# hamaadshah/gan_deeplearning4j

Measured on NVIDIA H100. Metric: images/sec (full G+D step), higher is better.
Workload: dtype bf16

## Files before the change

gan_deeplearning4j_b200/_lib.py:

```python
from __future__ import annotations

import ctypes as C
import os

_HERE = os.path.dirname(os.path.abspath(__file__))
LIB_PATH = os.path.join(_HERE, "lib", "libb200gan.so")
NAME_LEN = 64


class B200GanError(RuntimeError):
    def __init__(self, code, msg):
        super().__init__(f"libb200gan error {code}: {msg}")
        self.code = code


class LayerDesc(C.Structure):
    _fields_ = [("type", C.c_int32), ("name", C.c_char * NAME_LEN), ("n_in", C.c_int32), ("n_out", C.c_int32),
                ("k_h", C.c_int32), ("k_w", C.c_int32), ("s_h", C.c_int32), ("s_w", C.c_int32), ("p_h", C.c_int32), ("p_w", C.c_int32),
                ("has_bias", C.c_int32), ("act", C.c_int32), ("act_alpha", C.c_float), ("updater", C.c_int32),
                ("lr", C.c_float), ("beta1", C.c_float), ("beta2", C.c_float), ("eps", C.c_float), ("l2", C.c_float),
                ("bn_decay", C.c_float), ("bn_eps", C.c_float), ("pre_h", C.c_int32), ("pre_w", C.c_int32), ("pre_c", C.c_int32),
                ("loss", C.c_int32), ("frozen", C.c_int32)]


class NetConfig(C.Structure):
    _fields_ = [("in_h", C.c_int32), ("in_w", C.c_int32), ("in_c", C.c_int32), ("max_batch", C.c_int32), ("precision", C.c_int32),
                ("grad_clip", C.c_float), ("xent_clip_eps", C.c_float), ("bn_groups", C.c_int32), ("seed", C.c_uint64)]


class GanConfig(C.Structure):
    _fields_ = [("fake_bn_train", C.c_int32), ("use_cuda_graph", C.c_int32)]


class LrSchedule(C.Structure):
    _fields_ = [("kind", C.c_int32), ("type", C.c_int32), ("initial", C.c_double), ("gamma", C.c_double), ("power", C.c_double),
                ("step", C.c_double), ("decay_rate", C.c_double), ("n_map", C.c_int32), ("map_keys", C.POINTER(C.c_int32)),
                ("map_values", C.POINTER(C.c_double))]


class ConvGeom(C.Structure):
    _fields_ = [(k, C.c_int32) for k in ("n", "h", "w", "c", "oh", "ow", "o", "kh", "kw", "sh", "sw", "ph", "pw")]


class TestConvOpts(C.Structure):
    _fields_ = [("epi", C.c_int32), ("act", C.c_int32), ("alpha", C.c_float), ("bias", C.POINTER(C.c_float)), ("scale", C.POINTER(C.c_float)),
                ("groups", C.c_int32), ("aux", C.POINTER(C.c_float)), ("aux2", C.POINTER(C.c_float)), ("stats", C.POINTER(C.c_double)), ("kernel", C.c_char * 64),
                ("bn", C.c_int32), ("max_ctas", C.c_int32), ("poison", C.c_int32), ("w_mn", C.c_int32), ("per_tap", C.c_int32), ("slab", C.c_int32),
                ("defer", C.c_int32), ("db", C.POINTER(C.c_float)), ("param_offset", C.c_int32), ("splits", C.c_int32)]


class EwReduceJob(C.Structure):
    _fields_ = [("n", C.c_int64), ("stride", C.c_int64), ("src_off", C.c_int64), ("dst_off", C.c_int64), ("splits", C.c_int32), ("wide", C.c_int32)]


class TestEwOpts(C.Structure):
    _fields_ = [("op", C.c_int32), ("n", C.c_int64), ("rows", C.c_int32), ("cols", C.c_int32), ("groups", C.c_int32), ("splits", C.c_int32),
                ("stride", C.c_int64)] + [(k, C.c_int32) for k in ("N", "H", "W", "C", "KH", "KW", "SH", "SW", "act")] + [
                ("alpha", C.c_float), ("clip_eps", C.c_float), ("offset", C.c_int32), ("in_place", C.c_int32), ("accumulate", C.c_int32),
                ("poison", C.c_int32), ("n_jobs", C.c_int32), ("jobs", C.POINTER(EwReduceJob)), ("n_seg", C.c_int32),
                ("seg_off", C.POINTER(C.c_int64)), ("seg_len", C.POINTER(C.c_int64)), ("seg_coef", C.POINTER(C.c_float)), ("sumsq", C.c_double),
                ("kernel", C.c_char * 64), ("loss", C.c_int32)]


class TestPoolOpts(C.Structure):
    _fields_ = [("op", C.c_int32), ("pool", C.c_int32), ("pnorm", C.c_float)] + [
                (k, C.c_int32) for k in ("N", "H", "W", "C", "KH", "KW", "SH", "SW", "PH", "PW", "offset", "poison")] + [
                ("kernel", C.c_char * 64), ("splits", C.c_int32)]


_vp, _i32, _i64, _fp = C.c_void_p, C.c_int32, C.c_int64, C.POINTER(C.c_float)
_pvp = C.POINTER(C.c_void_p)

PROTOTYPES = {
    "b2g_version": (_i32, []),
    "b2g_ctx_create": (_i32, [_i32, _pvp]),
    "b2g_ctx_destroy": (_i32, [_vp]),
    "b2g_last_error": (C.c_char_p, []),
    "b2g_sync": (_i32, [_vp]),
    "b2g_launch_count": (_i32, [_vp, C.POINTER(C.c_uint64)]),
    "b2g_timer_start": (_i32, [_vp]),
    "b2g_timer_stop_ms": (_i32, [_vp, _fp]),
    "b2g_flush_l2": (_i32, [_vp]),
    "b2g_device_info": (_i32, [_vp, C.POINTER(_i32), C.POINTER(_i32), C.POINTER(_i32), C.POINTER(C.c_uint64)]),
    "b2g_net_create": (_i32, [_vp, C.POINTER(NetConfig), C.POINTER(LayerDesc), _i32, _pvp]),
    "b2g_net_destroy": (_i32, [_vp]),
    "b2g_net_num_params": (_i32, [_vp, C.POINTER(_i64)]),
    "b2g_net_output_size": (_i32, [_vp, C.POINTER(_i64)]),
    "b2g_net_layer_output_size": (_i32, [_vp, _i32, C.POINTER(_i64)]),
    "b2g_net_set_param": (_i32, [_vp, C.c_char_p, C.c_char_p, _fp, _i64]),
    "b2g_net_get_param": (_i32, [_vp, C.c_char_p, C.c_char_p, _fp, _i64]),
    "b2g_net_get_params": (_i32, [_vp, _fp, _i64]),
    "b2g_net_set_params": (_i32, [_vp, _fp, _i64]),
    "b2g_net_get_gradients": (_i32, [_vp, _fp, _i64]),
    "b2g_net_updater_state_size": (_i32, [_vp, C.POINTER(_i64)]),
    "b2g_net_get_updater_state": (_i32, [_vp, _fp, _i64]),
    "b2g_net_set_updater_state": (_i32, [_vp, _fp, _i64]),
    "b2g_net_output": (_i32, [_vp, _fp, _i32, _i32, _fp]),
    "b2g_net_get_activation": (_i32, [_vp, _i32, _i32, _fp]),
    "b2g_net_compute_gradient_and_score": (_i32, [_vp, _fp, _fp, _i32, _fp]),
    "b2g_net_get_input_gradient": (_i32, [_vp, _i32, _fp]),
    "b2g_net_fit": (_i32, [_vp, _fp, _fp, _i32, _fp]),
    "b2g_net_get_iteration": (_i32, [_vp, C.POINTER(_i64)]),
    "b2g_net_set_iteration": (_i32, [_vp, _i64]),
    "b2g_net_get_dropout_pass": (_i32, [_vp, C.POINTER(_i64)]),
    "b2g_net_set_dropout_pass": (_i32, [_vp, _i64]),
    "b2g_net_set_gradient_normalization": (_i32, [_vp, _i32, C.c_float]),
    "b2g_net_set_lr_schedule": (_i32, [_vp, C.c_char_p, C.POINTER(LrSchedule)]),
    "b2g_net_get_learning_rate": (_i32, [_vp, C.c_char_p, _fp]),
    "b2g_net_get_epoch": (_i32, [_vp, C.POINTER(_i64)]),
    "b2g_net_set_epoch": (_i32, [_vp, _i64]),
    "b2g_net_simt_gemm_calls": (_i32, [_vp, C.POINTER(C.c_uint64)]),
    "b2g_gan_create": (_i32, [_vp, _vp, C.POINTER(GanConfig), _pvp]),
    "b2g_gan_destroy": (_i32, [_vp]),
    "b2g_gan_step": (_i32, [_vp, _fp, _fp, _fp, _fp, _fp, _fp, _i32, _fp]),
    "b2g_gan_upload": (_i32, [_vp, _fp, _fp, _fp, _fp, _fp, _fp, _i32]),
    "b2g_gan_step_resident": (_i32, [_vp, _i32]),
    "b2g_gan_read_losses": (_i32, [_vp, _fp]),
    "b2g_gan_last_step_ms": (_i32, [_vp, _fp]),
    "b2g_comm_unique_id": (_i32, [_vp]),
    "b2g_ctx_comm_init": (_i32, [_vp, _i32, _i32, _vp]),
    "b2g_ctx_comm_destroy": (_i32, [_vp]),
    "b2g_net_set_grad_allreduce": (_i32, [_vp, _i32]),
    "b2g_net_average_parameters": (_i32, [_vp]),
    "b2g_net_set_sync_bn": (_i32, [_vp, _i32]),
    "b2g_net_set_grad_payload_bf16": (_i32, [_vp, _i32]),
    "b2g_net_enable_p2p_allreduce": (_i32, [_vp, C.POINTER(C.c_int32)]),
    "b2g_ctx_allreduce_test": (_i32, [_vp, _fp, _i64]),
    "b2g_test_conv": (_i32, [_vp, _i32, _i32, _i32, C.POINTER(ConvGeom), _fp, _fp, _fp, _i32, _fp]),
    "b2g_test_hbm_kernels": (_i32, [_vp, _i32, _i32, _i32, _fp]),
    "b2g_test_conv_ex": (_i32, [_vp, _i32, _i32, _i32, C.POINTER(ConvGeom), _fp, _fp, _fp, _i32, _fp, C.POINTER(TestConvOpts)]),
    "b2g_test_bn": (_i32, [_vp, _i32, _i32, _i32, _i32, _i32, _fp, _fp, _fp, _fp, _fp, _fp, _i32, C.c_float, C.c_float, C.c_float,
                           _i32, _fp, _fp, _fp, _fp, _fp, _fp, _fp, _fp]),
    "b2g_test_net_shadow": (_i32, [_vp, _i32, _i32, _fp, _i64]),
    "b2g_test_dropout": (_i32, [_vp, _i32, C.c_uint64, _i32, _i32, _i64, _i32, _i32, _i32, _i32, C.c_float, _fp, _fp, _fp, _fp]),
    "b2g_test_ew": (_i32, [_vp, _i32, C.POINTER(TestEwOpts), _fp, _fp, _fp, _fp, _fp]),
    "b2g_test_pool": (_i32, [_vp, _i32, C.POINTER(TestPoolOpts), _fp, _fp, _fp, _fp, _fp]),
}

_lib = None


def load():
    global _lib
    if _lib is not None:
        return _lib
    if not os.path.exists(LIB_PATH):
        raise B200GanError(-7, f"{LIB_PATH} is missing: build it with `make` (nvcc, sm_90a). There is no CPU fallback.")
    lib = C.CDLL(LIB_PATH, mode=C.RTLD_GLOBAL)
    for name, (res, args) in PROTOTYPES.items():
        fn = getattr(lib, name)
        fn.restype, fn.argtypes = res, args
    _lib = lib
    return lib


def check(code):
    if code != 0:
        raise B200GanError(code, load().b2g_last_error().decode(errors="replace"))
```

gan_deeplearning4j_b200/csrc/engine.cu:

```cuda
#include <cuda_runtime.h>
#include <dlfcn.h>
#include <math.h>
#include <stdarg.h>
#include <stdio.h>
#include <stdlib.h>
#include <string.h>

#include <algorithm>
#include <string>
#include <vector>

#include "../../include/b200gan.h"
#include "kernels.h"

using namespace b2g;

static thread_local char g_err[1024] = "";
static int32_t fail(int32_t code, const char* fmt, ...) {
  va_list ap; va_start(ap, fmt); vsnprintf(g_err, sizeof(g_err), fmt, ap); va_end(ap); return code;
}
#define CU(call) do { cudaError_t e_ = (call); if (e_ != cudaSuccess) return fail(B2G_ERR_CUDA, "%s:%d %s -> %s", __FILE__, __LINE__, #call, cudaGetErrorString(e_)); } while (0)
#define B2(call) do { int32_t r_ = (call); if (r_ != 0) return r_; } while (0)
#define CHECK_KERNELS() CU(cudaGetLastError())

// ... 1202 lines not shown
}
static bool layer_has_lr(const b2g_net* n, int li) { return lr_segment(n, li) >= 0; }
static int32_t find_lr_layer(const b2g_net* n, const char* layer, int* li) {
  for (size_t i = 0; i < n->L.size(); ++i) if (!strncmp(n->L[i].d.name, layer, B2G_NAME_LEN)) {
    if (!layer_has_lr(n, (int)i)) return fail(B2G_ERR_ARG, "layer %s has no learning rate (frozen, no parameters, NoOp or AdaDelta)", layer);
    *li = (int)i; return 0;
  }
  return fail(B2G_ERR_ARG, "no layer named %s", layer);
}
static int32_t net_upload_schedules(b2g_net* n) {
  cudaStream_t s = n->ctx->stream;
  size_t nv = 0; for (auto& ls : n->layer_sched) nv += ls.vals.size();
  const size_t bytes = nv * (sizeof(double) + sizeof(int32_t));
  CU(cudaStreamSynchronize(s));
  if (bytes > n->sched_map_bytes) {
    if (n->sched_map) { cudaFree(n->sched_map); n->sched_map = nullptr; n->sched_map_bytes = 0; }
    cudaError_t e = cudaMalloc(&n->sched_map, bytes);
    if (e != cudaSuccess) { n->sched_map = nullptr; return fail(B2G_ERR_OOM, "cudaMalloc(%zu) failed: %s", bytes, cudaGetErrorString(e)); }
    n->sched_map_bytes = bytes;
  }
  std::vector<char> host(bytes); double* dv = (double*)n->sched_map; int32_t* dk = (int32_t*)((char*)n->sched_map + nv * sizeof(double));
  std::vector<UpdSched> per_layer(n->L.size()); size_t at = 0;
  for (size_t li = 0; li < n->L.size(); ++li) {
    const auto& ls = n->layer_sched[li]; per_layer[li] = ls.sc;
    if (ls.sc.kind == B2G_SCHED_MAP) {
      memcpy(host.data() + at * sizeof(double), ls.vals.data(), ls.vals.size() * sizeof(double));
      memcpy(host.data() + nv * sizeof(double) + at * sizeof(int32_t), ls.keys.data(), ls.keys.size() * sizeof(int32_t));
      per_layer[li].vals = dv + at; per_layer[li].keys = dk + at; at += ls.vals.size();
    }
  }
  std::vector<UpdSched> seg(n->segs.size()); bool on = false;
  for (size_t i = 0; i < n->segs.size(); ++i) { seg[i] = per_layer[n->seg_layer[i]]; on = on || seg[i].kind != B2G_SCHED_NONE; }
  if (bytes) CU(cudaMemcpyAsync(n->sched_map, host.data(), bytes, cudaMemcpyHostToDevice, s));
  if (!seg.empty()) CU(cudaMemcpyAsync(n->sched_dev, seg.data(), sizeof(UpdSched) * seg.size(), cudaMemcpyHostToDevice, s));
  CU(cudaStreamSynchronize(s));
  n->sched_on = on; ++n->settings_gen;
  return 0;
}
extern "C" int32_t b2g_net_set_lr_schedule(b2g_net* n, const char* layer, const b2g_lr_schedule* s) {
  if (!n) return fail(B2G_ERR_ARG, "null"); CU(cudaSetDevice(n->ctx->device));
  b2g_net::LayerSched ls;
  if (s && s->kind != B2G_SCHED_NONE) {
    if (s->kind < B2G_SCHED_EXPONENTIAL || s->kind > B2G_SCHED_MAP) return fail(B2G_ERR_ARG, "unknown schedule kind %d (PolySchedule is not supported)", s->kind);
    if (s->type != B2G_SCHED_ITERATION && s->type != B2G_SCHED_EPOCH) return fail(B2G_ERR_ARG, "unknown schedule type %d", s->type);
    if (!std::isfinite(s->initial) || !std::isfinite(s->gamma) || !std::isfinite(s->power) || !std::isfinite(s->step) || !std::isfinite(s->decay_rate))
      return fail(B2G_ERR_ARG, "schedule parameters must be finite");
    if (s->kind == B2G_SCHED_STEP && !(s->step > 0.0)) return fail(B2G_ERR_ARG, "StepSchedule step %g: must be > 0", s->step);
    if (s->kind == B2G_SCHED_INVERSE && s->gamma < 0.0) return fail(B2G_ERR_ARG, "InverseSchedule gamma %g: must be >= 0", s->gamma);
    UpdSched& sc = ls.sc; sc.kind = s->kind; sc.type = s->type;
    sc.initial = s->initial; sc.gamma = s->gamma; sc.power = s->power; sc.step = s->step; sc.decay = s->decay_rate;
    if (s->kind == B2G_SCHED_MAP) {
      if (s->n_map < 1 || !s->map_keys || !s->map_values) return fail(B2G_ERR_ARG, "MapSchedule needs at least one entry");
      bool has0 = false;
      for (int j = 0; j < s->n_map; ++j) {
        if (j > 0 && s->map_keys[j] <= s->map_keys[j - 1]) return fail(B2G_ERR_ARG, "MapSchedule keys must strictly increase");
        if (!std::isfinite(s->map_values[j])) return fail(B2G_ERR_ARG, "MapSchedule values must be finite");
        has0 = has0 || s->map_keys[j] == 0;
      }
      if (!has0) return fail(B2G_ERR_ARG, "MapSchedule has no value for key 0");
      ls.keys.assign(s->map_keys, s->map_keys + s->n_map); ls.vals.assign(s->map_values, s->map_values + s->n_map); sc.n_map = s->n_map;
    }
  }
  if (layer) { int li = 0; B2(find_lr_layer(n, layer, &li)); n->layer_sched[li] = ls; }
  else for (size_t li = 0; li < n->L.size(); ++li) if (layer_has_lr(n, (int)li)) n->layer_sched[li] = ls;
  return net_upload_schedules(n);
}
extern "C" int32_t b2g_net_get_learning_rate(b2g_net* n, const char* layer, float* out) {
  if (!n || !layer || !out) return fail(B2G_ERR_ARG, "null"); CU(cudaSetDevice(n->ctx->device));
  int li = 0; B2(find_lr_layer(n, layer, &li));
  const int seg = lr_segment(n, li);
  k_sched_lr(n->segs_dev, n->sched_dev, seg, n->step_dev, n->epoch_dev, n->lr_out, n->ctx->stream); CHECK_KERNELS();
  CU(cudaMemcpyAsync(out, n->lr_out, sizeof(float), cudaMemcpyDeviceToHost, n->ctx->stream)); CU(cudaStreamSynchronize(n->ctx->stream));
  return 0;
}
extern "C" int32_t b2g_net_get_epoch(b2g_net* n, int64_t* out) {
  if (!n || !out) return fail(B2G_ERR_ARG, "null"); CU(cudaSetDevice(n->ctx->device));
  int64_t v = 0; CU(cudaMemcpyAsync(&v, n->epoch_dev, sizeof(v), cudaMemcpyDeviceToHost, n->ctx->stream)); CU(cudaStreamSynchronize(n->ctx->stream)); *out = v; return 0;
}
extern "C" int32_t b2g_net_set_epoch(b2g_net* n, int64_t epoch) {
  if (!n || epoch < 0) return fail(B2G_ERR_ARG, "bad epoch"); CU(cudaSetDevice(n->ctx->device));
  CU(cudaMemcpyAsync(n->epoch_dev, &epoch, sizeof(epoch), cudaMemcpyHostToDevice, n->ctx->stream)); CU(cudaStreamSynchronize(n->ctx->stream)); return 0;
}
extern "C" int32_t b2g_net_simt_gemm_calls(b2g_net* n, uint64_t* out) { if (!n || !out) return fail(B2G_ERR_ARG, "null"); *out = n->simt_gemm_calls; return 0; }

extern "C" int32_t b2g_comm_unique_id(void* id128) { if (!id128) return fail(B2G_ERR_ARG, "null"); B2(nccl_load()); NcclId id; NC(g_nccl.uid(&id)); memcpy(id128, &id, sizeof(id)); return 0; }
extern "C" int32_t b2g_ctx_comm_init(b2g_ctx* c, int32_t world, int32_t rank, const void* id128) {
  if (!c || !id128 || world < 1 || rank < 0 || rank >= world) return fail(B2G_ERR_ARG, "bad communicator arguments");
  B2(nccl_load()); CU(cudaSetDevice(c->device));
  NcclId id; memcpy(&id, id128, sizeof(id));
  NC(g_nccl.init(&c->comm, world, id, rank)); c->world = world; c->rank = rank; return 0;
}
extern "C" int32_t b2g_ctx_comm_destroy(b2g_ctx* c) { if (c && c->comm) { g_nccl.destroy(c->comm); c->comm = nullptr; c->world = 1; c->rank = 0; } return 0; }
extern "C" int32_t b2g_net_set_grad_allreduce(b2g_net* n, int32_t enabled) { if (!n) return fail(B2G_ERR_ARG, "null"); n->grad_allreduce = enabled != 0; return 0; }
extern "C" int32_t b2g_net_set_sync_bn(b2g_net* n, int32_t enabled) { if (!n) return fail(B2G_ERR_ARG, "null"); if (enabled && n->prec != PREC_BF16) return fail(B2G_ERR_UNSUPPORTED, "sync_bn rides on the fused BatchNorm path (BF16 nets)"); n->sync_bn = enabled != 0; return 0; }
extern "C" int32_t b2g_net_set_grad_payload_bf16(b2g_net* n, int32_t enabled) {
  if (!n) return fail(B2G_ERR_ARG, "null"); CU(cudaSetDevice(n->ctx->device));
  if (enabled && !n->ar_buf) B2(dalloc(n, &n->ar_buf, sizeof(__nv_bfloat16) * (size_t)n->n_params));
  n->ar_bf16 = enabled != 0; return 0;
}
extern "C" int32_t b2g_net_enable_p2p_allreduce(b2g_net* n, int32_t* enabled) {
  if (!n) return fail(B2G_ERR_ARG, "null"); b2g_ctx* c = n->ctx; CU(cudaSetDevice(c->device)); if (enabled) *enabled = 0;
  if (!c->comm || c->world < 2) return 0;
  if (c->world > 8 || !g_nccl.ag) return 0;
  cudaStream_t s = c->stream;
  if (!c->p2p_flags) { CU(cudaMalloc(&c->p2p_flags, 16 * sizeof(unsigned))); CU(cudaMalloc(&c->p2p_state, 2 * sizeof(unsigned)));
                       CU(cudaMemsetAsync(c->p2p_flags, 0, 16 * sizeof(unsigned), s)); CU(cudaMemsetAsync(c->p2p_state, 0, 2 * sizeof(unsigned), s)); CU(cudaStreamSynchronize(s)); }
  struct Pair { cudaIpcMemHandle_t flags, grads; };
  Pair mine; memset(&mine, 0, sizeof(mine)); float ok = 1.f;
  if (cudaIpcGetMemHandle(&mine.flags, c->p2p_flags) != cudaSuccess || cudaIpcGetMemHandle(&mine.grads, n->grads) != cudaSuccess) { cudaGetLastError(); ok = 0.f; }
  std::vector<Pair> all(c->world);
  char *d_send = nullptr, *d_recv = nullptr; float* d_ok = nullptr;
  CU(cudaMalloc(&d_send, sizeof(Pair))); CU(cudaMalloc(&d_recv, sizeof(Pair) * c->world)); CU(cudaMalloc(&d_ok, sizeof(float)));
  CU(cudaMemcpyAsync(d_send, &mine, sizeof(Pair), cudaMemcpyHostToDevice, s));
  NC(g_nccl.ag(d_send, d_recv, sizeof(Pair),  0, c->comm, s));
  CU(cudaMemcpyAsync(all.data(), d_recv, sizeof(Pair) * c->world, cudaMemcpyDeviceToHost, s)); CU(cudaStreamSynchronize(s));
  float* pg[8] = {}; unsigned* pf[8] = {};
  for (int r = 0; r < c->world && ok > 0.f; ++r) {
    if (r == c->rank) { pg[r] = n->grads; pf[r] = c->p2p_flags; continue; }
    void* q = nullptr;
    if (cudaIpcOpenMemHandle(&q, all[r].grads, cudaIpcMemLazyEnablePeerAccess) != cudaSuccess) { cudaGetLastError(); ok = 0.f; break; }
    pg[r] = (float*)q;
    if (c->p2p_flags_mapped) pf[r] = c->p2p_peer_flags[r];
    else { if (cudaIpcOpenMemHandle(&q, all[r].flags, cudaIpcMemLazyEnablePeerAccess) != cudaSuccess) { cudaGetLastError(); ok = 0.f; break; } pf[r] = (unsigned*)q; }
  }
  CU(cudaMemcpyAsync(d_ok, &ok, sizeof(float), cudaMemcpyHostToDevice, s)); NC(g_nccl.ar(d_ok, d_ok, 1, 7, 0, c->comm, s));
  float sum = 0.f; CU(cudaMemcpyAsync(&sum, d_ok, sizeof(float), cudaMemcpyDeviceToHost, s)); CU(cudaStreamSynchronize(s));
  cudaFree(d_send); cudaFree(d_recv); cudaFree(d_ok);
  if (sum < (float)c->world - 0.5f) {
    for (int r = 0; r < c->world; ++r) { if (r == c->rank) continue; if (pg[r]) cudaIpcCloseMemHandle(pg[r]); if (!c->p2p_flags_mapped && pf[r]) cudaIpcCloseMemHandle(pf[r]); }
    return 0;
  }
  for (int r = 0; r < c->world; ++r) { n->p2p_peer_grads[r] = pg[r]; c->p2p_peer_flags[r] = pf[r]; }
  c->p2p_flags_mapped = true; n->p2p = true; if (enabled) *enabled = 1;
  return 0;
}
extern "C" int32_t b2g_net_average_parameters(b2g_net* n) {
  if (!n) return fail(B2G_ERR_ARG, "null"); b2g_ctx* c = n->ctx; CU(cudaSetDevice(c->device));
  if (!c->comm || c->world == 1) return 0;
  const float inv = 1.0f / (float)c->world; cudaStream_t s = c->stream;
  float* bufs[4] = {n->params, n->st0, n->st1, n->st2};
  for (float* b : bufs) { if (!b) continue; NC(g_nccl.ar(b, b, (size_t)n->n_params, 7, 0, c->comm, s)); k_scale_f32(b, inv, (size_t)n->n_params, s); }
  net_refresh_shadow(n);
  CU(cudaStreamSynchronize(s)); return 0;
}
extern "C" int32_t b2g_ctx_allreduce_test(b2g_ctx* c, float* host, int64_t n) {
  if (!c || !host || n < 1) return fail(B2G_ERR_ARG, "null"); if (!c->comm) return fail(B2G_ERR_NCCL, "no communicator"); CU(cudaSetDevice(c->device));
  float* d = nullptr; CU(cudaMalloc(&d, sizeof(float) * n));
  CU(cudaMemcpyAsync(d, host, sizeof(float) * n, cudaMemcpyHostToDevice, c->stream));
  NC(g_nccl.ar(d, d, (size_t)n, 7, 0, c->comm, c->stream));
  CU(cudaMemcpyAsync(host, d, sizeof(float) * n, cudaMemcpyDeviceToHost, c->stream)); CU(cudaStreamSynchronize(c->stream)); cudaFree(d); return 0;
}

struct TcTestSchedule {
  TcTestSchedule(int bn, int max_ctas, int per_tap, int splits) { g_tc_test_bn = bn; g_tc_test_max_ctas = max_ctas; g_tc_test_per_tap = per_tap; g_tc_test_splits = splits; }
  ~TcTestSchedule() { reset(); }
  void reset() { g_tc_test_bn = 0; g_tc_test_max_ctas = 0; g_tc_test_per_tap = 0; g_tc_test_splits = 0; }
};
extern "C" int32_t b2g_test_conv_ex(b2g_ctx* c, int32_t kind, int32_t impl, int32_t precision, const b2g_conv_geom* gg, const float* a_host, const float* b_host, float* out, int32_t iters, float* ms_per_iter,
                                    b2g_test_conv_opts* opt) {
  if (!c || !gg || !a_host || !b_host || !out) return fail(B2G_ERR_ARG, "null"); CU(cudaSetDevice(c->device));
  cudaStream_t s = c->stream; int prec = precision == B2G_PREC_BF16 ? PREC_BF16 : PREC_F32; size_t ts = prec_size(prec);
  ConvGeom g{gg->n, gg->h, gg->w, gg->c, gg->oh, gg->ow, gg->o, gg->kh, gg->kw, gg->sh, gg->sw, gg->ph, gg->pw};
  size_t nx = (size_t)g.N * g.H * g.W * g.C, ny = (size_t)g.N * g.OH * g.OW * g.O, nw = (size_t)g.O * g.KH * g.KW * g.C;
  size_t na = kind == 1 ? ny : nx, nb = kind == 2 ? ny : nw, no = kind == 0 ? ny : kind == 1 ? nx : nw;
  const int oc = kind == 0 ? g.O : g.C;
  if (impl == 1) {
    if (prec != PREC_BF16 || !c->tc_ok) return fail(B2G_ERR_UNSUPPORTED, "tensor-core kernels need BF16 precision and a working tensor-map encoder");
    bool ok = kind == 0 ? tc_fprop_supported(g) : kind == 1 ? tc_dgrad_supported(g) : tc_wgrad_supported(g);
    if (!ok) return fail(B2G_ERR_UNSUPPORTED, "no tensor-core kernel for this shape");
  }
  const bool tc_conv = impl == 1 && kind != 2, ps = impl == 3 && kind == 1;
  const bool edge_fwd = impl == 3 && kind == 0, tc_wg = kind == 2 && (impl == 1 || impl == 3);
  const bool gemm = impl == 0 || impl == 2 || impl == 4;
  const bool gemm_epi = gemm && kind != 2 && !(impl == 4 && kind == 1 && !dense_small_k_supported(g));
  if (opt && gemm) {
    if (opt->epi || (!gemm_epi && (opt->bias || opt->scale || opt->act)))
      return fail(B2G_ERR_UNSUPPORTED, "impl %d kind %d: no epilogue (bias / activation: impl 0 / 2 kind 0 / 1, impl 4 kind 0 and the short-reduction kind 1; no fused BatchNorm epilogue)", impl, kind);
    if (opt->scale && impl != 0) return fail(B2G_ERR_UNSUPPORTED, "scale applies to the SIMT fprop / dgrad (impl 0) and the tensor-core kernels");
  }
  else if (opt && !tc_conv && !ps && !edge_fwd && (opt->epi || opt->bias || opt->scale || opt->act))
    return fail(B2G_ERR_UNSUPPORTED, "epilogue options apply to the tensor-core fprop / dgrad kernels (impl 1, kind 0 / 1), the tensor-core skinny-layer conv and pixel-shuffle deconv (impl 3, kind 0 / 1) and the SIMT / skinny-layer / dense kernels (impl 0 / 2 / 4)");
  if (opt && edge_fwd && (opt->epi || opt->scale)) return fail(B2G_ERR_UNSUPPORTED, "the tensor-core skinny-layer conv has bias and activation only");
  const int poff = opt ? opt->param_offset : 0;
  if (poff < 0 || (poff && !gemm && !tc_wg))
    return fail(B2G_ERR_UNSUPPORTED, "param_offset %d: applies to the SIMT / skinny-layer / dense kernels (impl 0 / 2 / 4) and the tensor-core weight gradients (kind 2, impl 1 / 3)", poff);
  if (opt && ps && (opt->scale || (opt->epi != EPI_PLAIN && opt->epi != EPI_ACTBWD)))
    return fail(B2G_ERR_UNSUPPORTED, "the pixel-shuffle deconv has bias, activation and the activation-backward epilogue only");
  const int force_bn = opt ? opt->bn : 0, max_ctas = opt ? opt->max_ctas : 0;
  const bool poison = opt && opt->poison, w_mn = opt && opt->w_mn, per_tap = opt && opt->per_tap;
  if (per_tap && !tc_conv) return fail(B2G_ERR_UNSUPPORTED, "per_tap applies to the tensor-core fprop / dgrad kernels (impl 1, kind 0 / 1)");
  if (force_bn && (!tc_conv || (force_bn != 64 && force_bn != 128) || oc % force_bn))
    return fail(B2G_ERR_UNSUPPORTED, "bn %d: the tensor-core fprop / dgrad tile is 64 or 128 columns and must divide the %d output channels", force_bn, oc);
  if (max_ctas < 0 || (max_ctas && !tc_conv && !ps && !edge_fwd))
    return fail(B2G_ERR_UNSUPPORTED, "max_ctas %d: a grid cap applies to tc_conv_kernel and tc_edge_conv_kernel launches only", max_ctas);
  const int force_splits = opt ? opt->splits : 0;
  if (force_splits < 0 || (force_splits && !tc_wg)) return fail(B2G_ERR_UNSUPPORTED, "splits %d: a forced split count applies to the tensor-core weight gradients (kind 2, impl 1 / 3)", force_splits);
  if (w_mn && (impl != 1 || kind != 0 || g.KH != 1 || g.KW != 1)) return fail(B2G_ERR_UNSUPPORTED, "w_mn: the [C][O] weight operand exists for the 1x1 tensor-core fprop only");
  const bool defer = opt && opt->defer; float* db_host = opt ? opt->db : nullptr;
  if (defer && !(kind == 2 && (impl == 1 || impl == 3))) return fail(B2G_ERR_UNSUPPORTED, "defer applies to the tensor-core weight gradients (kind 2, impl 1 / 3)");
  if (db_host && !(kind == 2 && impl == 3)) return fail(B2G_ERR_UNSUPPORTED, "db is the edge tensor-core weight gradient's bias column (kind 2, impl 3)");
  if (impl == 2 || impl == 3) {
    bool ok = kind == 0 ? edge_conv_small_cin_supported(g) : kind == 1 ? edge_deconv_small_c_supported(g) : edge_wgrad_small_cin_supported(g);
    if (impl == 3) ok = ok && prec == PREC_BF16 && c->tc_ok && (kind == 0 ? tc_edge_conv_supported(g) : kind == 1 ? tc_deconv_ps_supported(g) : tc_edge_wgrad_supported(g));
    if (ps) ok = prec == PREC_BF16 && c->tc_ok && tc_deconv_ps_supported(g);
    if (!ok) return fail(B2G_ERR_UNSUPPORTED, "no skinny-layer kernel (impl %d) for this shape", impl);
  }
  if (impl == 4 && !(dense_small_o_supported(g) || (dense_small_k_supported(g) && kind != 0))) return fail(B2G_ERR_UNSUPPORTED, "no dense kernel for this shape");
  float *fa = nullptr, *fb = nullptr, *fo = nullptr, *scratch = nullptr; void *ta = nullptr, *tb = nullptr, *to = nullptr; __nv_bfloat16* wps = nullptr;
  float *d_bias = nullptr, *d_scale = nullptr, *d_coef = nullptr, *d_auxf = nullptr; __nv_bfloat16 *d_aux = nullptr, *d_aux2 = nullptr; unsigned long long* d_acc = nullptr;
  size_t sc = std::max(std::max(std::max(k_simt_wgrad_scratch_floats(g), k_tc_wgrad_scratch_floats(g)), std::max(k_edge_wgrad_scratch_floats(g), k_tc_edge_wgrad_scratch_floats(g))), k_dense_small_o_wgrad_scratch_floats(g)) + 16;
  if (force_splits) sc = std::max(sc, (size_t)force_splits * (impl == 1 ? nw : (size_t)64 * 16 * g.C + 64) + 16);
  const size_t woff = (prec == PREC_F32 && kind != 2) ? (size_t)poff : 0, dwoff = kind == 2 ? (size_t)poff : 0;
  CU(cudaMalloc(&fa, 4 * na)); CU(cudaMalloc(&fb, 4 * nb)); CU(cudaMalloc(&fo, 4 * (no + dwoff))); CU(cudaMalloc(&scratch, 4 * sc));
  CU(cudaMalloc(&ta, ts * na)); CU(cudaMalloc(&tb, ts * nb + 4 * woff)); CU(cudaMalloc(&to, ts * no));
  float* const fres = fo + dwoff;
  void* const tbase = tb; tb = (float*)tb + woff;
  CU(cudaMemcpyAsync(fa, a_host, 4 * na, cudaMemcpyHostToDevice, s)); CU(cudaMemcpyAsync(fb, b_host, 4 * nb, cudaMemcpyHostToDevice, s));
  if (prec == PREC_BF16) { k_cast_f32_to_bf16(fa, (__nv_bfloat16*)ta, na, s); k_cast_f32_to_bf16(fb, (__nv_bfloat16*)tb, nb, s); }
  else { CU(cudaMemcpyAsync(ta, fa, 4 * na, cudaMemcpyDeviceToDevice, s)); CU(cudaMemcpyAsync(tb, fb, 4 * nb, cudaMemcpyDeviceToDevice, s)); }
  if (impl == 3 && kind == 1) { CU(cudaMalloc(&wps, 2 * k_tc_deconv_ps_weight_elems(g))); k_pack_deconv_ps(fb, wps, g.O, g.C, s); }
  float *d_db = nullptr, *dbres = nullptr; int db_written = 0;
  if (db_host) { CU(cudaMalloc(&d_db, 4 * ((size_t)g.O + dwoff))); dbres = d_db + dwoff; }
  ReduceList rl{}; ReduceList* prl = defer ? &rl : nullptr;
  TcEpi epi{}; const TcEpi* pe = nullptr; const float* bias = nullptr; int act = 0; float alpha = 0.f; int groups = 1;
  if (opt && (tc_conv || ps || edge_fwd)) {
    groups = opt->groups > 0 ? opt->groups : 1; act = opt->act; alpha = opt->alpha;
    if (opt->bias) { CU(cudaMalloc(&d_bias, 4 * oc)); CU(cudaMemcpyAsync(d_bias, opt->bias, 4 * oc, cudaMemcpyHostToDevice, s)); bias = d_bias; }
    if (opt->scale) { CU(cudaMalloc(&d_scale, 4 * oc)); CU(cudaMemcpyAsync(d_scale, opt->scale, 4 * oc, cudaMemcpyHostToDevice, s)); }
    epi.mode = opt->epi; epi.scale = d_scale; epi.imgs_per_group = g.N / groups; epi.act = opt->act; epi.alpha = opt->alpha;
    if (opt->epi == EPI_STATS || opt->epi == EPI_BNBWD) { CU(cudaMalloc(&d_acc, 8 * k_bn_acc_elems(oc, groups))); epi.acc = d_acc; }
    if (opt->epi == EPI_BNBWD || opt->epi == EPI_ACTBWD) {
      if (!opt->aux) return fail(B2G_ERR_ARG, "epilogue %d needs aux", opt->epi);
      CU(cudaMalloc(&d_auxf, 4 * no)); CU(cudaMalloc(&d_aux, 2 * no)); CU(cudaMemcpyAsync(d_auxf, opt->aux, 4 * no, cudaMemcpyHostToDevice, s)); k_cast_f32_to_bf16(d_auxf, d_aux, no, s); epi.aux = d_aux;
    }
    if (opt->epi == EPI_BNBWD) {
      if (!opt->aux2) return fail(B2G_ERR_ARG, "epilogue 2 needs aux2 (the BatchNorm input z)");
      CU(cudaMalloc(&d_coef, 4 * no)); CU(cudaMalloc(&d_aux2, 2 * no)); CU(cudaMemcpyAsync(d_coef, opt->aux2, 4 * no, cudaMemcpyHostToDevice, s)); k_cast_f32_to_bf16(d_coef, d_aux2, no, s); epi.aux2 = d_aux2;
    }
    if (opt->epi || opt->scale) pe = &epi;
  }
  if (opt && gemm_epi) {
    act = opt->act; alpha = opt->alpha;
    if (opt->bias) { CU(cudaMalloc(&d_bias, 4 * oc)); CU(cudaMemcpyAsync(d_bias, opt->bias, 4 * oc, cudaMemcpyHostToDevice, s)); bias = d_bias; }
    if (opt->scale) { CU(cudaMalloc(&d_scale, 4 * oc)); CU(cudaMemcpyAsync(d_scale, opt->scale, 4 * oc, cudaMemcpyHostToDevice, s)); }
  }
  cudaEvent_t e0, e1; CU(cudaEventCreate(&e0)); CU(cudaEventCreate(&e1));
  int reps = iters < 1 ? 1 : iters; int rc = 0;
  g_tc_last_kernel = ""; g_tc_last_slab = false; g_tc_last_splits = 0; g_gemm_last_kernel = ""; g_gemm_last_splits = 0;
  TcTestSchedule schedule(force_bn, max_ctas, per_tap, force_splits);
  for (int it = -1; it < reps; ++it) {
    if (it == 0) CU(cudaEventRecord(e0, s));
    if (d_acc) CU(cudaMemsetAsync(d_acc, 0, 8 * k_bn_acc_elems(oc, groups), s));
    if (poison) CU(cudaMemsetAsync(to, 0xFF, ts * no, s));
    if (poison && kind == 2) { CU(cudaMemsetAsync(fres, 0xFF, 4 * no, s)); CU(cudaMemsetAsync(scratch, 0xFF, 4 * sc, s)); }
    if (poison && dbres) CU(cudaMemsetAsync(dbres, 0xFF, 4 * (size_t)g.O, s));
    if (impl == 4) {
      const bool so = dense_small_o_supported(g);
      if (kind == 0) k_dense_small_o_fwd(prec, prec, g, ta, tb, bias, to, act, alpha, s);
      else if (kind == 1) { if (so && !bias && !act) k_dense_small_o_dgrad(prec, prec, g, ta, tb, to, s); else k_dense_small_k_dgrad(prec, prec, g, ta, tb, bias, to, act, alpha, s); }
      else { if (so) k_dense_small_o_wgrad(prec, g, ta, tb, fres, scratch, 0, s); else k_dense_small_k_wgrad(prec, g, ta, tb, fres, s); }
    }
    else if (impl >= 2) {
      if (kind == 0) { if (impl == 3) rc = k_tc_edge_conv(g, (const __nv_bfloat16*)ta, (const __nv_bfloat16*)tb, bias, (__nv_bfloat16*)to, act, alpha, s); else k_edge_conv_small_cin(prec, prec, g, ta, tb, bias, to, act, alpha, s); }
      else if (kind == 1) { if (impl == 3) rc = k_tc_deconv_ps(g, (const __nv_bfloat16*)ta, wps, bias, (__nv_bfloat16*)to, act, alpha, s, pe); else k_edge_deconv_small_c(prec, prec, g, ta, tb, bias, to, act, alpha, s); }
      else {
        if (impl == 3) { rc = k_tc_edge_wgrad(g, (const __nv_bfloat16*)ta, (const __nv_bfloat16*)tb, fres, dbres, scratch, sc, 0, s, prl); if (rc >= 0) { db_written = rc; rc = 0; } }
        else k_edge_wgrad_small_cin(prec, g, ta, tb, fres, scratch, 0, s);
      }
    }
    else if (kind == 0) { if (impl) rc = k_tc_fprop(g, (const __nv_bfloat16*)ta, (const __nv_bfloat16*)tb, bias, (__nv_bfloat16*)to, act, alpha, s, pe, w_mn ? 1 : 0); else k_simt_fprop(prec, prec, g, ta, tb, bias, to, act, alpha, s, d_scale); }
    else if (kind == 1) { if (impl) rc = k_tc_dgrad(g, (const __nv_bfloat16*)ta, (const __nv_bfloat16*)tb, bias, (__nv_bfloat16*)to, act, alpha, s, pe); else k_simt_dgrad(prec, prec, g, ta, tb, bias, to, act, alpha, s, d_scale); }
    else { if (impl) rc = k_tc_wgrad(g, (const __nv_bfloat16*)ta, (const __nv_bfloat16*)tb, fres, scratch, sc, 0, s, prl); else k_simt_wgrad(prec, g, ta, tb, fres, scratch, sc, 0, s); }
    if (rc) break;
    if (defer) {
      if (!rl.count) { rc = -4; break; }
      k_reduce_multi(rl, s); rl.count = 0;
    }
  }
  schedule.reset();
  CU(cudaEventRecord(e1, s));
  if (rc == -4) return fail(B2G_ERR_CUDA, "defer: the weight gradient queued no reduction");
  if (rc) return fail(B2G_ERR_CUDA, "tensor-core kernel launch failed (%d)", rc);
  if (opt) {
    strncpy(opt->kernel, gemm ? g_gemm_last_kernel : g_tc_last_kernel, sizeof(opt->kernel) - 1); opt->kernel[sizeof(opt->kernel) - 1] = 0; opt->slab = g_tc_last_slab;
    opt->splits = gemm ? g_gemm_last_splits : tc_wg ? g_tc_last_splits : 0;
  }
  if (d_db) {
    if (!db_written) { cudaFree(d_db); return fail(B2G_ERR_UNSUPPORTED, "the edge weight gradient produces no bias column for C = %d", g.C); }
    CU(cudaMemcpyAsync(db_host, dbres, 4 * (size_t)g.O, cudaMemcpyDeviceToHost, s));
  }
  if (kind != 2) { if (prec == PREC_BF16) {  k_nhwc_to_nchw_f32(prec, to, fo, 1, 1, (int)no, s); } else CU(cudaMemcpyAsync(fo, to, 4 * no, cudaMemcpyDeviceToDevice, s)); }
  CU(cudaMemcpyAsync(out, fres, 4 * no, cudaMemcpyDeviceToHost, s));
  CU(cudaStreamSynchronize(s)); CHECK_KERNELS();
  if (d_acc && opt && opt->stats) {
    std::vector<long long> h(k_bn_acc_elems(oc, groups)); CU(cudaMemcpy(h.data(), d_acc, 8 * h.size(), cudaMemcpyDeviceToHost));
    for (int gi = 0; gi < groups; ++gi) for (int st = 0; st < 2; ++st) for (int ch = 0; ch < oc; ++ch)
      opt->stats[((size_t)gi * 2 + st) * oc + ch] = (double)h[((size_t)(gi * 2 + st) * 2 + 0) * oc + ch] / 1024.0 + (double)h[((size_t)(gi * 2 + st) * 2 + 1) * oc + ch] / 1152921504606846976.0;
  }
  float ms = 0.f; CU(cudaEventElapsedTime(&ms, e0, e1)); if (ms_per_iter) *ms_per_iter = ms / reps;
  cudaEventDestroy(e0); cudaEventDestroy(e1);
  cudaFree(fa); cudaFree(fb); cudaFree(fo); cudaFree(scratch); cudaFree(ta); cudaFree(tbase); cudaFree(to); if (wps) cudaFree(wps); if (d_db) cudaFree(d_db);
  if (d_bias) cudaFree(d_bias); if (d_scale) cudaFree(d_scale); if (d_coef) cudaFree(d_coef); if (d_auxf) cudaFree(d_auxf); if (d_aux) cudaFree(d_aux); if (d_aux2) cudaFree(d_aux2); if (d_acc) cudaFree(d_acc);
  return 0;
}
extern "C" int32_t b2g_test_conv(b2g_ctx* c, int32_t kind, int32_t impl, int32_t precision, const b2g_conv_geom* gg, const float* a_host, const float* b_host, float* out, int32_t iters, float* ms_per_iter) {
  return b2g_test_conv_ex(c, kind, impl, precision, gg, a_host, b_host, out, iters, ms_per_iter, nullptr);
}

extern "C" int32_t b2g_test_bn(b2g_ctx* c, int32_t precision, int32_t path, int32_t groups, int32_t rows, int32_t C, const float* x, const float* eps_out,
                               const float* gamma, const float* beta, const float* run_mean, const float* run_var, int32_t act, float alpha, float eps, float decay,
                               int32_t want_param_grads, float* y, float* eps_in, float* g_gamma, float* g_beta, float* g_mean, float* g_var, float* mean, float* invstd) {
  if (!c || !x || !eps_out || !gamma || !beta || !run_mean || !run_var || !y || !eps_in || !g_gamma || !g_beta || !g_mean || !g_var || !mean || !invstd) return fail(B2G_ERR_ARG, "null");
  if (groups < 1 || rows < 1 || C < 1 || path < 0 || path > 2) return fail(B2G_ERR_ARG, "bad BatchNorm test arguments");
  const int prec = precision == B2G_PREC_BF16 ? PREC_BF16 : PREC_F32;
  if (path != 0 && !k_bn_vec_ok(prec, C)) return fail(B2G_ERR_UNSUPPORTED, "the accumulator BatchNorm kernels need bf16 and C %% 8 == 0 with 256 %% (C/8) == 0 (C = %d)", C);
  CU(cudaSetDevice(c->device)); cudaStream_t s = c->stream;
  const size_t n = (size_t)groups * rows * C, gc = (size_t)groups * C, ts = prec_size(prec);
  std::vector<void*> mem;
  auto alloc = [&](void** p, size_t bytes) -> int32_t { *p = nullptr; CU(cudaMalloc(p, bytes)); mem.push_back(*p); return 0; };
  auto release = [&]() { for (void* p : mem) cudaFree(p); mem.clear(); };
  float *fx, *fe, *fo, *d_par, *d_grad, *d_stat, *scratch, *coef, *unit; void *tx, *te, *ty, *tei; unsigned long long* acc;
  int32_t r = 0;
  if ((r = alloc((void**)&fx, 4 * n)) || (r = alloc((void**)&fe, 4 * n)) || (r = alloc((void**)&fo, 4 * n)) || (r = alloc(&tx, ts * n)) || (r = alloc(&te, ts * n)) ||
      (r = alloc(&ty, ts * n)) || (r = alloc(&tei, ts * n)) || (r = alloc((void**)&d_par, 4 * 4 * (size_t)C)) || (r = alloc((void**)&d_grad, 4 * 4 * (size_t)C)) ||
      (r = alloc((void**)&d_stat, 4 * 2 * gc)) || (r = alloc((void**)&scratch, 4 * k_bn_scratch_floats(C, groups))) || (r = alloc((void**)&coef, 4 * 4 * gc)) ||
      (r = alloc((void**)&unit, 4 * 4 * gc)) || (r = alloc((void**)&acc, 8 * 2 * k_bn_acc_elems(C, groups)))) { release(); return r; }
  float *d_gamma = d_par, *d_beta = d_par + C, *d_rm = d_par + 2 * C, *d_rv = d_par + 3 * C;
  float *d_gg = d_grad, *d_gb = d_grad + C, *d_gm = d_grad + 2 * C, *d_gv = d_grad + 3 * C, *d_mean = d_stat, *d_is = d_stat + gc;
  unsigned long long *acc_f = acc, *acc_b = acc + k_bn_acc_elems(C, groups);
  auto up = [&](float* d, const float* h, size_t k) { return cudaMemcpyAsync(d, h, 4 * k, cudaMemcpyHostToDevice, s); };
  if (up(fx, x, n) || up(fe, eps_out, n) || up(d_gamma, gamma, C) || up(d_beta, beta, C) || up(d_rm, run_mean, C) || up(d_rv, run_var, C) ||
      up(d_gg, g_gamma, C) || up(d_gb, g_beta, C) || cudaMemsetAsync(acc, 0, 8 * 2 * k_bn_acc_elems(C, groups), s)) { release(); return fail(B2G_ERR_CUDA, "BatchNorm test upload failed"); }
  if (prec == PREC_BF16) { k_cast_f32_to_bf16(fx, (__nv_bfloat16*)tx, n, s); k_cast_f32_to_bf16(fe, (__nv_bfloat16*)te, n, s); }
  else { cudaMemcpyAsync(tx, fx, 4 * n, cudaMemcpyDeviceToDevice, s); cudaMemcpyAsync(te, fe, 4 * n, cudaMemcpyDeviceToDevice, s); }
  const int want = want_param_grads ? 1 : 0;
  if (path == 0) {
    k_bn_stats(prec, tx, rows, C, groups, scratch, d_mean, d_is, eps, d_rm, d_rv, d_gm, d_gv, decay, s);
    k_bn_apply(prec, tx, ty, rows, C, groups, d_mean, d_is, d_gamma, d_beta, act, alpha, s);
    k_bn_bwd(prec, tx, te, tei, rows, C, groups, d_mean, d_is, d_gamma, d_beta, act, alpha, scratch, d_gg, d_gb, want, s);
  } else {
    k_bn_stats_acc(tx, rows, C, groups, acc_f, s);
    k_bn_apply_acc(tx, ty, rows, C, groups, acc_f, d_gamma, d_beta, act, alpha, eps, coef, d_rm, d_rv, d_gm, d_gv, decay, s, 1);
    if (path == 1) k_bn_bwd_stats_acc(tx, te, rows, C, groups, coef, act, alpha, acc_b, s);
    else {
      for (int g = 0; g < groups; ++g) for (int k = 0; k < 4; ++k) k_fill_f32(unit + (size_t)(g * 4 + k) * C, (k == 0 || k == 3) ? 1.f : 0.f, C, s);
      k_bn_bwd_stats_acc(tx, te, rows, C, groups, unit, ACT_IDENTITY, 0.f, acc_b, s);
    }
    k_bn_bwd_apply_acc(tx, te, tei, rows, C, groups, coef, act, alpha, path == 2 ? 1 : 0, acc_b, d_gg, d_gb, want, s, 1);
    for (int g = 0; g < groups; ++g) {
      cudaMemcpyAsync(d_mean + (size_t)g * C, coef + (size_t)(g * 4 + 2) * C, 4 * C, cudaMemcpyDeviceToDevice, s);
      cudaMemcpyAsync(d_is + (size_t)g * C, coef + (size_t)(g * 4 + 3) * C, 4 * C, cudaMemcpyDeviceToDevice, s);
    }
  }
  auto down = [&](float* h, const void* t) -> int32_t {
    k_nhwc_to_nchw_f32(prec, t, fo, 1, 1, (int)n, s); CU(cudaMemcpyAsync(h, fo, 4 * n, cudaMemcpyDeviceToHost, s)); CU(cudaStreamSynchronize(s)); return 0;
  };
  if ((r = down(y, ty)) || (r = down(eps_in, tei))) { release(); return r; }
  cudaError_t e = cudaSuccess;
  float* hs[6] = {g_gamma, g_beta, g_mean, g_var, mean, invstd}; const float* ds[6] = {d_gg, d_gb, d_gm, d_gv, d_mean, d_is}; const size_t ks[6] = {(size_t)C, (size_t)C, (size_t)C, (size_t)C, gc, gc};
  for (int k = 0; k < 6 && e == cudaSuccess; ++k) e = cudaMemcpyAsync(hs[k], ds[k], 4 * ks[k], cudaMemcpyDeviceToHost, s);
  if (e == cudaSuccess) e = cudaStreamSynchronize(s);
  if (e == cudaSuccess) e = cudaGetLastError();
  release();
  if (e != cudaSuccess) return fail(B2G_ERR_CUDA, "BatchNorm test: %s", cudaGetErrorString(e));
  return 0;
}

extern "C" int32_t b2g_test_dropout(b2g_ctx* c, int32_t precision, uint64_t seed, int32_t layer, int32_t rank, int64_t pass, int32_t rows, int32_t h, int32_t w, int32_t ch,
                                    float p, const float* x, const float* dy, float* y, float* dx) {
  if (!c || !x || !dy || !y || !dx) return fail(B2G_ERR_ARG, "null");
  if (!(p > 0.f && p <= 1.f)) return fail(B2G_ERR_ARG, "dropout retain probability %g outside (0, 1]", (double)p);
  if (rows < 1 || h < 1 || w < 1 || ch < 1 || layer < 0 || layer > 0xffff || rank < 0 || rank > 0xffff || pass < 0) return fail(B2G_ERR_ARG, "bad dropout test arguments");
  const size_t n = (size_t)rows * h * w * ch;
  if (n > 0x7fffffff) return fail(B2G_ERR_UNSUPPORTED, "the dropout test hook takes at most 2^31 - 1 elements (%zu)", n);
  const int prec = precision == B2G_PREC_BF16 ? PREC_BF16 : PREC_F32; const size_t ts = prec_size(prec);
  CU(cudaSetDevice(c->device)); cudaStream_t s = c->stream;
  std::vector<void*> mem;
  auto alloc = [&](void** q, size_t bytes) -> int32_t { *q = nullptr; CU(cudaMalloc(q, bytes)); mem.push_back(*q); return 0; };
  auto release = [&]() { for (void* q : mem) cudaFree(q); mem.clear(); };
  float *fx, *fe; void *tx, *te, *ty; uint32_t* mask; unsigned long long* dpass; unsigned* ticket; int32_t r = 0;
  if ((r = alloc((void**)&fx, 4 * n)) || (r = alloc((void**)&fe, 4 * n)) || (r = alloc(&tx, ts * n)) || (r = alloc(&te, ts * n)) || (r = alloc(&ty, ts * n)) ||
      (r = alloc((void**)&mask, 4 * ((n + 31) / 32))) || (r = alloc((void**)&dpass, sizeof(unsigned long long))) || (r = alloc((void**)&ticket, sizeof(unsigned)))) { release(); return r; }
  const unsigned long long p0 = (unsigned long long)pass;
  cudaError_t e = cudaMemcpyAsync(fx, x, 4 * n, cudaMemcpyHostToDevice, s);
  if (e == cudaSuccess) e = cudaMemcpyAsync(fe, dy, 4 * n, cudaMemcpyHostToDevice, s);
  if (e == cudaSuccess) e = cudaMemcpyAsync(dpass, &p0, sizeof(p0), cudaMemcpyHostToDevice, s);
  if (e == cudaSuccess) e = cudaMemsetAsync(ticket, 0, sizeof(unsigned), s);
  if (e != cudaSuccess) { release(); return fail(B2G_ERR_CUDA, "dropout test upload: %s", cudaGetErrorString(e)); }
  if (prec == PREC_BF16) { k_cast_f32_to_bf16(fx, (__nv_bfloat16*)tx, n, s); k_cast_f32_to_bf16(fe, (__nv_bfloat16*)te, n, s); }
  else { cudaMemcpyAsync(tx, fx, 4 * n, cudaMemcpyDeviceToDevice, s); cudaMemcpyAsync(te, fe, 4 * n, cudaMemcpyDeviceToDevice, s); }
  const DropoutArgs a = make_dropout_args(seed, layer, rank, p);
  k_dropout_fwd(prec, tx, ty, mask, n, a, dpass, ticket, 1, s);
  k_dropout_bwd(prec, te, te, mask, n, a.scale, s);
  unsigned long long p1 = 0;
  k_nhwc_to_nchw_f32(prec, ty, fx, 1, 1, (int)n, s);
  k_nhwc_to_nchw_f32(prec, te, fe, 1, 1, (int)n, s);
  e = cudaMemcpyAsync(y, fx, 4 * n, cudaMemcpyDeviceToHost, s);
  if (e == cudaSuccess) e = cudaMemcpyAsync(dx, fe, 4 * n, cudaMemcpyDeviceToHost, s);
  if (e == cudaSuccess) e = cudaMemcpyAsync(&p1, dpass, sizeof(p1), cudaMemcpyDeviceToHost, s);
  if (e == cudaSuccess) e = cudaStreamSynchronize(s);
  if (e == cudaSuccess) e = cudaGetLastError();
  release();
  if (e != cudaSuccess) return fail(B2G_ERR_CUDA, "dropout test: %s", cudaGetErrorString(e));
  if (p1 != p0 + 1) return fail(B2G_ERR_CUDA, "dropout test: the forward left the pass counter at %llu, expected %llu", p1, p0 + 1);
  return 0;
}

namespace {
struct EwMem {
  std::vector<void*> v;
  ~EwMem() { for (void* p : v) cudaFree(p); }
};
}
enum { EW_POOL2D = 100, EW_GLOBAL_POOL = 101 };
static int32_t test_ew_impl(b2g_ctx* c, int32_t precision, b2g_test_ew_opts* o, b2g_test_pool_opts* po, const float* in0, const float* in1, float* out0,
                            float* out1, float* out2) {
  if (!c || !o) return fail(B2G_ERR_ARG, "null");
  const int prec = precision == B2G_PREC_BF16 ? PREC_BF16 : PREC_F32; const size_t ts = prec_size(prec);
  const int off = o->offset;
  if (off < 0 || off > 64) return fail(B2G_ERR_ARG, "offset %d outside [0, 64]", off);
  if (o->poison && o->accumulate) return fail(B2G_ERR_ARG, "poison would overwrite the initial destination accumulate adds to");
  CU(cudaSetDevice(c->device)); cudaStream_t s = c->stream;
  EwMem mem;
  auto dev = [&](size_t count, size_t es, void** p) -> int32_t { void* b = nullptr; CU(cudaMalloc(&b, es * (count + off) + 16)); mem.v.push_back(b); *p = (char*)b + es * off; return 0; };
  auto upF = [&](const float* h, size_t count, float** p) -> int32_t {
    B2(dev(count, 4, (void**)p)); if (h) CU(cudaMemcpyAsync(*p, h, 4 * count, cudaMemcpyHostToDevice, s)); return 0; };
  auto upT = [&](const float* h, size_t count, void** p) -> int32_t {
    B2(dev(count, ts, p)); if (!h) return 0;
    if (prec == PREC_F32) { CU(cudaMemcpyAsync(*p, h, 4 * count, cudaMemcpyHostToDevice, s)); return 0; }
    float* f = nullptr; CU(cudaMalloc(&f, 4 * count)); mem.v.push_back(f);
    CU(cudaMemcpyAsync(f, h, 4 * count, cudaMemcpyHostToDevice, s)); k_cast_f32_to_bf16(f, (__nv_bfloat16*)*p, count, s); return 0; };
  auto downF = [&](float* h, const float* d, size_t count) -> int32_t { if (h) CU(cudaMemcpyAsync(h, d, 4 * count, cudaMemcpyDeviceToHost, s)); return 0; };
  auto downT = [&](float* h, const void* d, size_t count) -> int32_t {
    if (!h) return 0;
    float* f = nullptr; CU(cudaMalloc(&f, 4 * count)); mem.v.push_back(f);
    k_nhwc_to_nchw_f32(prec, d, f, 1, 1, (int)count, s); CU(cudaMemcpyAsync(h, f, 4 * count, cudaMemcpyDeviceToHost, s)); return 0; };
  auto poison = [&](void* d, size_t bytes) -> int32_t { if (o->poison) CU(cudaMemsetAsync(d, 0xFF, bytes, s)); return 0; };
// ... 249 lines not shown
```

gan_deeplearning4j_b200/csrc/kernels.h:

```cpp
#pragma once
#include <cuda_runtime.h>
#include <cuda_bf16.h>
#include <stdint.h>

namespace b2g {

enum Prec { PREC_F32 = 0, PREC_BF16 = 1 };
enum Act { ACT_IDENTITY = 0, ACT_TANH = 1, ACT_SIGMOID = 2, ACT_RELU = 3, ACT_LRELU = 4,
           ACT_ELU = 5, ACT_SELU = 6, ACT_SOFTPLUS = 7, ACT_SOFTSIGN = 8, ACT_HARDTANH = 9, ACT_HARDSIGMOID = 10, ACT_RELU6 = 11, ACT_SWISH = 12,
           ACT_CUBE = 13, ACT_RATIONALTANH = 14, ACT_RECTIFIEDTANH = 15, ACT_THRESHOLDEDRELU = 16, ACT_EXT_FIRST = ACT_ELU, ACT_EXT_LAST = ACT_THRESHOLDEDRELU };
enum Loss { LOSS_MSE = 2, LOSS_L1 = 3, LOSS_L2 = 4, LOSS_MAE = 5, LOSS_HINGE = 6, LOSS_SQUARED_HINGE = 7, LOSS_WASSERSTEIN = 8 };

inline size_t prec_size(int prec) { return prec == PREC_F32 ? 4 : 2; }

struct ConvGeom {
  int N, H, W, C;
  int OH, OW, O;
  int KH, KW, SH, SW, PH, PW;
};

extern uint64_t g_launch_count;
extern const char* g_ew_last_kernel;
int device_sm_count();

void k_nchw_f32_to_nhwc(int prec, const float* src, void* dst, int N, int C, int HW, cudaStream_t s);
void k_nhwc_to_nchw_f32(int prec, const void* src, float* dst, int N, int C, int HW, cudaStream_t s);
void k_permute(int prec, const void* src, void* dst, int N, int C, int HW, int to_nhwc, cudaStream_t s);
void k_cast_f32_to_bf16(const float* src, __nv_bfloat16* dst, size_t n, cudaStream_t s);

void k_bn_stats(int prec, const void* x, int rows_per_group, int C, int groups, float* scratch,
                float* mean, float* invstd, float eps,
                const float* run_mean, const float* run_var, float* g_mean, float* g_var, float decay, cudaStream_t s);
size_t k_bn_scratch_floats(int C, int groups);
void k_bn_fold(const float* run_mean, const float* run_var, const float* gamma, const float* beta, const float* conv_bias, int C, float eps, float* scale, float* shift, cudaStream_t s);
void k_bn_prep_infer(const float* run_mean, const float* run_var, int C, int groups, float eps, float* mean, float* invstd, cudaStream_t s);
void k_bn_apply(int prec, const void* x, void* y, int rows_per_group, int C, int groups, const float* mean, const float* invstd,
                const float* gamma, const float* beta, int act, float alpha, cudaStream_t s);
void k_bn_bwd(int prec, const void* x, const void* eps_out, void* eps_in, int rows_per_group, int C, int groups,
              const float* mean, const float* invstd, const float* gamma, const float* beta, int act, float alpha,
              float* scratch, float* g_gamma, float* g_beta, int want_param_grads, cudaStream_t s);

bool k_bn_vec_ok(int prec, int C);
size_t k_bn_acc_elems(int C, int groups);
void k_bn_stats_acc(const void* x, int rows_per_group, int C, int groups, unsigned long long* acc, cudaStream_t s);
void k_bn_apply_acc(const void* x, void* y, int rows_per_group, int C, int groups, const unsigned long long* acc, const float* gamma, const float* beta,
                    int act, float alpha, float eps, float* coef, const float* run_mean, const float* run_var, float* g_mean, float* g_var, float decay, cudaStream_t s, int replicas = 1);
void k_bn_bwd_stats_acc(const void* x, const void* eps_out, int rows_per_group, int C, int groups, const float* coef, int act, float alpha, unsigned long long* acc, cudaStream_t s);
void k_bn_bwd_apply_acc(const void* x, const void* eps_out, void* eps_in, int rows_per_group, int C, int groups, const float* coef, int act, float alpha, int premul,
                        const unsigned long long* acc, float* g_gamma, float* g_beta, int want_param_grads, cudaStream_t s, int replicas = 1);

void k_act_fwd(int prec, const void* x, void* y, size_t n, int act, float alpha, cudaStream_t s);
void k_act_bwd_from_output(int prec, const void* a, const void* eps_out, void* eps_in, size_t n, int act, float alpha, cudaStream_t s);
bool act_ext_kind(int act);
void k_act_ext_fwd(int prec, int act, float alpha, const void* z, void* a, size_t n, cudaStream_t s);
void k_act_ext_bwd(int prec, int act, float alpha, const void* z, void* eps, size_t n, cudaStream_t s);
void k_maxpool_fwd(int prec, const void* x, void* y, uint8_t* argmax, int N, int H, int W, int C, int OH, int OW, int KH, int KW, int SH, int SW, cudaStream_t s);
void k_maxpool_bwd(int prec, const void* eps_out, const uint8_t* argmax, void* eps_in, int N, int H, int W, int C, int OH, int OW, int KH, int KW, int SH, int SW, cudaStream_t s);
void k_upsample_fwd(int prec, const void* x, void* y, int N, int H, int W, int C, int f, cudaStream_t s);
void k_upsample_bwd(int prec, const void* eps_out, void* eps_in, int N, int H, int W, int C, int f, cudaStream_t s);

enum Pool { POOL_MAX = 0, POOL_AVG = 1, POOL_SUM = 2, POOL_PNORM = 3 };
void k_pool2d_fwd(int prec, int kind, int pn, const void* x, void* y, int N, int H, int W, int C, int OH, int OW, int KH, int KW, int SH, int SW, int PH, int PW,
                  cudaStream_t s);
void k_pool2d_bwd(int prec, int kind, int pn, const void* eps_out, const void* x, const void* y, void* eps_in, int N, int H, int W, int C, int OH, int OW, int KH,
                  int KW, int SH, int SW, int PH, int PW, cudaStream_t s);
int k_global_pool_splits(int prec, int N, int HW, int C, int vec);
size_t k_global_pool_partial_elems(int prec, int max_rows, int HW, int C);
void k_global_pool_fwd(int prec, int kind, int pn, const void* x, void* y, int32_t* idx, int N, int HW, int C, float* part, int32_t* part_idx, unsigned* ticket,
                       cudaStream_t s);
void k_global_pool_bwd(int prec, int kind, int pn, const void* eps_out, const void* x, const void* y, const int32_t* idx, void* eps_in, int N, int HW, int C,
                       cudaStream_t s);
extern int g_pool_last_splits;

struct DropoutArgs { uint64_t seed; uint32_t tag; uint32_t threshold; float scale; int keep_all; };
void k_dropout_fwd(int prec, const void* x, void* y, uint32_t* mask, size_t n, const DropoutArgs& a, unsigned long long* pass, unsigned* ticket, int bump_pass, cudaStream_t s);
void k_dropout_bwd(int prec, const void* eps_out, void* eps_in, const uint32_t* mask, size_t n, float scale, cudaStream_t s);

void k_xent(int prec, const void* z, const float* y, void* dz, float* loss_sums, int rows_per_group, int groups, float clip_eps, cudaStream_t s);
void k_sigmoid_out(int prec, const void* z, void* p, size_t n, cudaStream_t s);
void k_softmax_xent(int prec, const void* z, const float* y, void* dz, void* p_out, float* loss_sums, int rows, int K, cudaStream_t s);
int k_loss_blocks(size_t n_per_group, int groups);
void k_loss(int prec, int loss, int act, float alpha, const void* z, const float* y, void* dz, float* loss_sums, int rows_per_group, int n_out, int groups,
            double* partial, unsigned* ticket, cudaStream_t s);

void k_colsum(int prec, const void* x, int rows, int C, float* scratch, float* out, int accumulate, cudaStream_t s);
size_t k_colsum_scratch_floats(int C);
void k_sumsq_segments(const float* p, const int64_t* seg_off, const int64_t* seg_len, const float* seg_coef, int nseg, double* out, cudaStream_t s);
void k_reduce_splits(const float* src, float* dst, size_t n, int splits, size_t stride, int accumulate, cudaStream_t s);
struct ReduceJob { const float* src; float* dst; int64_t n, stride; int splits, blocks; };
struct ReduceList { static const int MAX_JOBS = 24; ReduceJob jobs[MAX_JOBS]; int count; };
void reduce_list_push(ReduceList* rl, const float* src, float* dst, int64_t n, int splits, int64_t stride);
void k_reduce_multi(const ReduceList& rl, cudaStream_t s);

struct UpdSeg {
  int64_t off, len;
  int kind;
  float lr, b1, b2, eps;
  float l2;
  float clip;
  int div_mb;
  int64_t off_bf, off_ps;
  int ps_O, ps_C;
};
struct UpdSched {
  int kind, type;
  int n_map;
  double initial, gamma, power, step, decay;
  const int32_t* keys; const double* vals;
};
void k_updater(float* params, const float* grads, float* st0, float* st1, float* st2, const UpdSeg* segs_dev, const int32_t* chunk_seg_dev,
               const int64_t* chunk_off_dev, int nchunks, float inv_mb, float inv_world, int* step_dev , unsigned* ticket,
               __nv_bfloat16* shadow, const float* gn_mult, const UpdSched* sched, const int64_t* epoch_dev, bool ext, cudaStream_t s);
void k_sched_lr(const UpdSeg* segs_dev, const UpdSched* sched, int seg, const int* step_dev, const int64_t* epoch_dev, float* out, cudaStream_t s);
static const int UPD_CHUNK = 4096;

struct GnGroup { int32_t chunk_begin, chunk_end, seg_begin, seg_end; };
void k_gradnorm(const float* grads, const UpdSeg* segs_dev, const int32_t* chunk_seg_dev, const int64_t* chunk_off_dev, int nchunks,
                const GnGroup* groups_dev, int ngroups, int clip, float threshold, float inv_mb, float inv_world, double* partial, unsigned* ticket,
                float* mult, cudaStream_t s);
void k_fill_f32(float* p, float v, size_t n, cudaStream_t s);
void k_scale_f32(float* p, float v, size_t n, cudaStream_t s);
struct P2pArgs { float* grads[8]; unsigned* flags[8]; int rank, world; size_t n; unsigned* state; };
void k_p2p_allreduce(const P2pArgs& a, cudaStream_t s);

void k_simt_fprop(int prec, int wprec, const ConvGeom& g, const void* x, const void* w, const float* bias, void* out, int act, float alpha, cudaStream_t s, const float* scale = nullptr);
void k_simt_dgrad(int prec, int wprec, const ConvGeom& g, const void* dy, const void* w, const float* bias, void* dx, int act, float alpha, cudaStream_t s, const float* scale = nullptr);
void k_simt_wgrad(int prec, const ConvGeom& g, const void* x, const void* dy, float* dw, float* scratch, size_t scratch_floats, int accumulate, cudaStream_t s);
size_t k_simt_wgrad_scratch_floats(const ConvGeom& g);
extern const char* g_gemm_last_kernel;
extern int g_gemm_last_splits;

bool edge_deconv_small_c_supported(const ConvGeom& g);
bool edge_conv_small_cin_supported(const ConvGeom& g);
bool edge_wgrad_small_cin_supported(const ConvGeom& g);
bool dense_small_o_supported(const ConvGeom& g);
void k_edge_deconv_small_c(int prec, int wprec, const ConvGeom& g, const void* dy, const void* w, const float* bias, void* dx, int act, float alpha, cudaStream_t s);
void k_edge_conv_small_cin(int prec, int wprec, const ConvGeom& g, const void* x, const void* w, const float* bias, void* out, int act, float alpha, cudaStream_t s);
void k_edge_wgrad_small_cin(int prec, const ConvGeom& g, const void* x, const void* dy, float* dw, float* scratch, int accumulate, cudaStream_t s);
size_t k_edge_wgrad_scratch_floats(const ConvGeom& g);
void k_dense_small_o_fwd(int prec, int wprec, const ConvGeom& g, const void* x, const void* w, const float* bias, void* out, int act, float alpha, cudaStream_t s);
void k_dense_small_o_dgrad(int prec, int wprec, const ConvGeom& g, const void* dy, const void* w, void* dx, cudaStream_t s);
void k_dense_small_o_wgrad(int prec, const ConvGeom& g, const void* x, const void* dy, float* dw, float* scratch, int accumulate, cudaStream_t s);
size_t k_dense_small_o_wgrad_scratch_floats(const ConvGeom& g);
bool dense_small_k_supported(const ConvGeom& g);
void k_dense_small_k_dgrad(int prec, int wprec, const ConvGeom& g, const void* dy, const void* w, const float* bias, void* dx, int act, float alpha, cudaStream_t s);
void k_dense_small_k_wgrad(int prec, const ConvGeom& g, const void* x, const void* dy, float* dw, cudaStream_t s);

bool tc_fprop_supported(const ConvGeom& g);
bool tc_dgrad_supported(const ConvGeom& g);
bool tc_wgrad_supported(const ConvGeom& g);
int  tc_init();
extern const char* g_tc_last_kernel;
extern int g_tc_test_bn, g_tc_test_max_ctas;
extern int g_tc_test_per_tap;
extern bool g_tc_last_slab;
extern int g_tc_test_splits, g_tc_last_splits;
enum { EPI_PLAIN = 0, EPI_STATS = 1, EPI_BNBWD = 2, EPI_ACTBWD = 3 };
struct TcEpi {
  int mode;
  const float* scale;
  unsigned long long* acc;
  int imgs_per_group;
  const __nv_bfloat16* aux;
  const __nv_bfloat16* aux2;
  int act; float alpha;
};
int k_tc_fprop(const ConvGeom& g, const __nv_bfloat16* x, const __nv_bfloat16* w, const float* bias, __nv_bfloat16* out, int act, float alpha, cudaStream_t s, const TcEpi* epi = nullptr, int w_mn = 0);
int k_tc_dgrad(const ConvGeom& g, const __nv_bfloat16* dy, const __nv_bfloat16* w, const float* bias, __nv_bfloat16* dx, int act, float alpha, cudaStream_t s, const TcEpi* epi = nullptr);
int k_tc_wgrad(const ConvGeom& g, const __nv_bfloat16* x, const __nv_bfloat16* dy, float* dw, float* scratch, size_t scratch_floats, int accumulate, cudaStream_t s, ReduceList* defer = nullptr);
size_t k_tc_wgrad_scratch_floats(const ConvGeom& g);
bool tc_deconv_ps_shape(const ConvGeom& g);
bool tc_deconv_ps_supported(const ConvGeom& g);
size_t k_tc_deconv_ps_weight_elems(const ConvGeom& g);
void k_pack_deconv_ps(const float* w, __nv_bfloat16* wps, int O, int C, cudaStream_t s);
bool tc_edge_conv_supported(const ConvGeom& g);
bool tc_edge_wgrad_supported(const ConvGeom& g);
size_t k_tc_edge_wgrad_scratch_floats(const ConvGeom& g);
int k_tc_edge_conv(const ConvGeom& g, const __nv_bfloat16* x, const __nv_bfloat16* w, const float* bias, __nv_bfloat16* out, int act, float alpha, cudaStream_t s);
int k_tc_edge_wgrad(const ConvGeom& g, const __nv_bfloat16* x, const __nv_bfloat16* dy, float* dw, float* db, float* scratch, size_t scratch_floats, int accumulate, cudaStream_t s, ReduceList* defer = nullptr);
int k_tc_deconv_ps(const ConvGeom& g, const __nv_bfloat16* dy, const __nv_bfloat16* wps, const float* bias, __nv_bfloat16* dx, int act, float alpha, cudaStream_t s, const TcEpi* epi = nullptr);

}
```

gan_deeplearning4j_b200/csrc/kernels_tc.cu:

```cuda
#include <cuda.h>
#include <stdio.h>
#include <stdlib.h>
#include <algorithm>

#include "common.cuh"
#include "kernels.h"

namespace b2g {

typedef CUresult (*PFN_encodeTiled)(CUtensorMap*, CUtensorMapDataType, cuuint32_t, void*, const cuuint64_t*, const cuuint64_t*, const cuuint32_t*,
                                    const cuuint32_t*, CUtensorMapInterleave, CUtensorMapSwizzle, CUtensorMapL2promotion, CUtensorMapFloatOOBfill);
static PFN_encodeTiled g_encode = nullptr;

int tc_init() {
  if (g_encode) return 0;
  void* fn = nullptr; cudaDriverEntryPointQueryResult q;
  if (cudaGetDriverEntryPoint("cuTensorMapEncodeTiled", &fn, cudaEnableDefault, &q) != cudaSuccess || !fn || q != cudaDriverEntryPointSuccess) return -1;
  g_encode = (PFN_encodeTiled)fn; return 0;
}

static int make_map_bf16(CUtensorMap* m, const void* base, int rank, const cuuint64_t* dims, const cuuint64_t* strides_bytes, const cuuint32_t* box, const cuuint32_t* estr) {
  if (!g_encode) return -1;
  CUresult r = g_encode(m, CU_TENSOR_MAP_DATA_TYPE_BFLOAT16, (cuuint32_t)rank, const_cast<void*>(base), dims, strides_bytes, box, estr, CU_TENSOR_MAP_INTERLEAVE_NONE,
                        CU_TENSOR_MAP_SWIZZLE_128B, CU_TENSOR_MAP_L2_PROMOTION_L2_256B, CU_TENSOR_MAP_FLOAT_OOB_FILL_NONE);
  if (r != CUDA_SUCCESS) { fprintf(stderr, "[b200gan] cuTensorMapEncodeTiled failed: %d (rank %d)\n", (int)r, rank); return -1; }
  return 0;
}

__device__ __forceinline__ uint32_t smem_u32(const void* p) { return (uint32_t)__cvta_generic_to_shared(p); }
__device__ __forceinline__ void mbar_init(uint32_t bar, uint32_t count) { asm volatile("mbarrier.init.shared::cta.b64 [%0], %1;" ::"r"(bar), "r"(count)); }
__device__ __forceinline__ void fence_mbar_init() { asm volatile("fence.mbarrier_init.release.cluster;" ::: "memory"); }
__device__ __forceinline__ void mbar_expect_tx(uint32_t bar, uint32_t bytes) { asm volatile("mbarrier.arrive.expect_tx.shared::cta.b64 _, [%0], %1;" ::"r"(bar), "r"(bytes) : "memory"); }
__device__ __forceinline__ void mbar_arrive(uint32_t bar) { asm volatile("mbarrier.arrive.shared::cta.b64 _, [%0];" ::"r"(bar) : "memory"); }
__device__ int g_tc_timeout_flag = 0;
__device__ __forceinline__ void mbar_wait(uint32_t bar, uint32_t parity) {
  uint32_t done = 0;
  for (uint32_t it = 0; it < (1u << 26); ++it) {
    asm volatile("{\n\t.reg .pred p;\n\tmbarrier.try_wait.parity.shared::cta.b64 p, [%1], %2;\n\tselp.u32 %0, 1, 0, p;\n\t}" : "=r"(done) : "r"(bar), "r"(parity) : "memory");
    if (done) return;
  }
  g_tc_timeout_flag = 1; __trap();
}
__device__ __forceinline__ void tma_load_4d(uint32_t dst, const CUtensorMap* map, uint32_t bar, int c0, int c1, int c2, int c3) {
  asm volatile("cp.async.bulk.tensor.4d.shared::cluster.global.tile.mbarrier::complete_tx::bytes [%0], [%1, {%3, %4, %5, %6}], [%2];"
               ::"r"(dst), "l"(map), "r"(bar), "r"(c0), "r"(c1), "r"(c2), "r"(c3) : "memory");
}
__device__ __forceinline__ void tma_load_3d(uint32_t dst, const CUtensorMap* map, uint32_t bar, int c0, int c1, int c2) {
  asm volatile("cp.async.bulk.tensor.3d.shared::cluster.global.tile.mbarrier::complete_tx::bytes [%0], [%1, {%3, %4, %5}], [%2];"
               ::"r"(dst), "l"(map), "r"(bar), "r"(c0), "r"(c1), "r"(c2) : "memory");
}
__device__ __forceinline__ void tma_load_2d(uint32_t dst, const CUtensorMap* map, uint32_t bar, int c0, int c1) {
  asm volatile("cp.async.bulk.tensor.2d.shared::cluster.global.tile.mbarrier::complete_tx::bytes [%0], [%1, {%3, %4}], [%2];"
               ::"r"(dst), "l"(map), "r"(bar), "r"(c0), "r"(c1) : "memory");
}
__device__ __forceinline__ bool elect_one_sync() {
  uint32_t pred = 0;
  asm volatile("{\n\t.reg .pred P1;\n\t.reg .b32 rx;\n\telect.sync rx|P1, %1;\n\t@P1 mov.s32 %0, 1;\n\t}" : "+r"(pred) : "r"(0xffffffffu));
  return pred != 0;
}
__device__ __forceinline__ void prefetch_map(const CUtensorMap* map) { asm volatile("prefetch.tensormap [%0];" ::"l"(map) : "memory"); }
__device__ __forceinline__ void fence_proxy_async_smem() { asm volatile("fence.proxy.async.shared::cta;" ::: "memory"); }

__device__ __forceinline__ uint64_t gmma_desc(uint32_t saddr, uint32_t lbo_bytes) {
  return (uint64_t)((saddr & 0x3FFFFu) >> 4) | ((uint64_t)((lbo_bytes >> 4) & 0x3FFF) << 16) | ((uint64_t)(1024 >> 4) << 32) | (1ull << 62);
}
__device__ __forceinline__ uint64_t desc_kmajor_sw128(uint32_t saddr) { return gmma_desc(saddr, 16); }
__device__ __forceinline__ uint64_t desc_mnmajor_sw128(uint32_t saddr, uint32_t lbo_bytes) { return gmma_desc(saddr, lbo_bytes); }

__device__ __forceinline__ void wg_fence() { asm volatile("wgmma.fence.sync.aligned;" ::: "memory"); }
__device__ __forceinline__ void wg_commit() { asm volatile("wgmma.commit_group.sync.aligned;" ::: "memory"); }
template <int N>
__device__ __forceinline__ void wg_wait() { asm volatile("wgmma.wait_group.sync.aligned %0;" ::"n"(N) : "memory"); }

template <int TA, int TB>
__device__ __forceinline__ void wgmma_n64(float (&d)[32], uint64_t da, uint64_t db) {
  asm volatile(
      "wgmma.mma_async.sync.aligned.m64n64k16.f32.bf16.bf16 "
      "{%0, %1, %2, %3, %4, %5, %6, %7, %8, %9, %10, %11, %12, %13, %14, %15, %16, %17, %18, %19, %20, %21, %22, %23, %24, %25, %26, %27, %28, %29, %30, %31}, "
      "%32, %33, 1, 1, 1, %34, %35;"
      : "+f"(d[0]), "+f"(d[1]), "+f"(d[2]), "+f"(d[3]), "+f"(d[4]), "+f"(d[5]), "+f"(d[6]), "+f"(d[7]), "+f"(d[8]), "+f"(d[9]), "+f"(d[10]),
        "+f"(d[11]), "+f"(d[12]), "+f"(d[13]), "+f"(d[14]), "+f"(d[15]), "+f"(d[16]), "+f"(d[17]), "+f"(d[18]), "+f"(d[19]), "+f"(d[20]),
        "+f"(d[21]), "+f"(d[22]), "+f"(d[23]), "+f"(d[24]), "+f"(d[25]), "+f"(d[26]), "+f"(d[27]), "+f"(d[28]), "+f"(d[29]), "+f"(d[30]), "+f"(d[31])
      : "l"(da), "l"(db), "n"(TA), "n"(TB));
}
template <int TA, int TB>
__device__ __forceinline__ void wgmma_n128(float (&d0)[32], float (&d1)[32], uint64_t da, uint64_t db) {
  asm volatile(
      "wgmma.mma_async.sync.aligned.m64n128k16.f32.bf16.bf16 "
      "{%0, %1, %2, %3, %4, %5, %6, %7, %8, %9, %10, %11, %12, %13, %14, %15, %16, %17, %18, %19, %20, %21, %22, %23, %24, %25, %26, %27, %28, %29, %30, %31, %32, %33, %34, %35, %36, %37, %38, %39, %40, %41, %42, %43, %44, %45, %46, %47, %48, %49, %50, %51, %52, %53, %54, %55, %56, %57, %58, %59, %60, %61, %62, %63}, "
      "%64, %65, 1, 1, 1, %66, %67;"
      : "+f"(d0[0]), "+f"(d0[1]), "+f"(d0[2]), "+f"(d0[3]), "+f"(d0[4]), "+f"(d0[5]), "+f"(d0[6]), "+f"(d0[7]), "+f"(d0[8]), "+f"(d0[9]), "+f"(d0[10]), "+f"(d0[11]), "+f"(d0[12]), "+f"(d0[13]), "+f"(d0[14]), "+f"(d0[15]), "+f"(d0[16]), "+f"(d0[17]), "+f"(d0[18]), "+f"(d0[19]), "+f"(d0[20]), "+f"(d0[21]), "+f"(d0[22]), "+f"(d0[23]), "+f"(d0[24]), "+f"(d0[25]), "+f"(d0[26]), "+f"(d0[27]), "+f"(d0[28]), "+f"(d0[29]), "+f"(d0[30]), "+f"(d0[31]),
        "+f"(d1[0]), "+f"(d1[1]), "+f"(d1[2]), "+f"(d1[3]), "+f"(d1[4]), "+f"(d1[5]), "+f"(d1[6]), "+f"(d1[7]), "+f"(d1[8]), "+f"(d1[9]), "+f"(d1[10]), "+f"(d1[11]), "+f"(d1[12]), "+f"(d1[13]), "+f"(d1[14]), "+f"(d1[15]), "+f"(d1[16]), "+f"(d1[17]), "+f"(d1[18]), "+f"(d1[19]), "+f"(d1[20]), "+f"(d1[21]), "+f"(d1[22]), "+f"(d1[23]), "+f"(d1[24]), "+f"(d1[25]), "+f"(d1[26]), "+f"(d1[27]), "+f"(d1[28]), "+f"(d1[29]), "+f"(d1[30]), "+f"(d1[31])
      : "l"(da), "l"(db), "n"(TA), "n"(TB));
}
__device__ __forceinline__ void wgmma_n16(float (&d)[8], uint64_t da, uint64_t db) {
  asm volatile(
      "wgmma.mma_async.sync.aligned.m64n16k16.f32.bf16.bf16 {%0, %1, %2, %3, %4, %5, %6, %7}, %8, %9, 1, 1, 1, 0, 0;"
      : "+f"(d[0]), "+f"(d[1]), "+f"(d[2]), "+f"(d[3]), "+f"(d[4]), "+f"(d[5]), "+f"(d[6]), "+f"(d[7])
      : "l"(da), "l"(db));
}



struct TcConvParams {
  int mode;
  int Nt, Ht, Wt;
  int GH, GW;
  int tiles_y;
  int taps_h, taps_w;
  int slab_bytes;
  int a_wg_bytes;
  int a_tap_bytes;
  int chunks;
  int KW, SH, SW, PH, PW;
  int OC;
  int outH, outW;
  int b_mn;
  const float* bias; const float* scale; int act; float alpha;
  __nv_bfloat16* out;
  int epi;
  unsigned long long* acc;
  int imgs_per_group;
  const __nv_bfloat16* aux;
  const __nv_bfloat16* aux2;
  int tiles_m, tiles_n, phases;
};

static constexpr int TC_THREADS = 384;
static constexpr int TC_CONV_THREADS = 640;
static constexpr int SLAB_ROWS = 144;
template <int BN, int STAGES, int EPI = EPI_PLAIN, bool SLAB = false>
struct TcSmem {
  static constexpr int A_BYTES = (SLAB ? SLAB_ROWS : 128) * 128;
  static constexpr int B_BYTES = (SLAB ? 2 : 1) * BN * 128;
  static constexpr int STAGE_BYTES = A_BYTES + B_BYTES;
  static constexpr int RING_BYTES = STAGES * STAGE_BYTES;
  static constexpr int ACC_PITCH = BN + 4;
  static constexpr int PARK_BYTES = 128 * ACC_PITCH * 4;
  static constexpr int PARKS = BN >= 128 ? 1 : 2;
  static constexpr int PARK_OFF = RING_BYTES;
  static constexpr int BAR_OFF = PARK_OFF + PARKS * PARK_BYTES;
  static constexpr int STAT_OFF = BAR_OFF + 256;
  static constexpr int STG_OFF = STAT_OFF + ((EPI == EPI_STATS || EPI == EPI_BNBWD) ? 4 * 2 * BN * 4 : 0);
  static constexpr int TOTAL = STG_OFF + (BN >= 32 ? 8 * 2048 : 0) + 1024;
  static_assert(TOTAL <= 227 * 1024, "one CTA per SM must fit the shared memory of an sm_90 SM");
};

__device__ __forceinline__ void epi_bar_sync() { asm volatile("bar.sync 1, 256;" ::: "memory"); }
template <int N> __device__ __forceinline__ void setmaxnreg_inc() { asm volatile("setmaxnreg.inc.sync.aligned.u32 %0;" ::"n"(N)); }
template <int N> __device__ __forceinline__ void setmaxnreg_dec() { asm volatile("setmaxnreg.dec.sync.aligned.u32 %0;" ::"n"(N)); }

template <int OFF>
__device__ __forceinline__ void warp_colsum_level(float (&a)[32], int lane) {
  const bool up = (lane & OFF) != 0;
#pragma unroll
  for (int j = 0; j < OFF; ++j) {
    const float lo = a[j], hi = a[j + OFF];
    const float send = up ? lo : hi, keep = up ? hi : lo;
    a[j] = keep + __shfl_xor_sync(0xffffffffu, send, OFF);
  }
  if constexpr (OFF > 1) warp_colsum_level<OFF / 2>(a, lane);
}
__device__ __forceinline__ void warp_colsum32(float (&a)[32], int lane) { warp_colsum_level<16>(a, lane); }

template <int BN, int EPI, bool AFFINE>
__device__ __forceinline__ void epi_tile(const TcConvParams& p, const float* srow, size_t roff, int nb0, int group, float* sst, uint4* stg, int q, int lane, int ep_tid,
                                         int c_beg, int c_end) {
  constexpr bool stats = EPI == EPI_STATS || EPI == EPI_BNBWD;
  const bool has_bias = p.bias != nullptr;
  const int sub = lane >> 2, cq = lane & 3, sx = (lane >> 1) & 3;
  size_t roff_i[4];
#pragma unroll
  for (int i = 0; i < 4; ++i) roff_i[i] = __shfl_sync(0xffffffffu, (unsigned long long)roff, i * 8 + sub) + cq * 8;
#pragma unroll 1
  for (int c0 = c_beg; c0 < c_end; c0 += 32) {
    uint32_t v[32];
    uint4 gy[4], gz[4], ax[4], az[4];
    if constexpr (EPI >= EPI_BNBWD) {
#pragma unroll
      for (int i = 0; i < 4; ++i) gy[i] = *reinterpret_cast<const uint4*>(p.aux + roff_i[i] + c0);
    }
    if constexpr (EPI == EPI_BNBWD) {
#pragma unroll
      for (int i = 0; i < 4; ++i) gz[i] = *reinterpret_cast<const uint4*>(p.aux2 + roff_i[i] + c0);
    }
    if constexpr (EPI >= EPI_BNBWD) {
#pragma unroll
      for (int i = 0; i < 4; ++i) { const int r = i * 8 + sub; stg[r * 4 + (cq ^ ((r >> 1) & 3))] = gy[i]; }
      __syncwarp();
#pragma unroll
      for (int j = 0; j < 4; ++j) ax[j] = stg[lane * 4 + (j ^ sx)];
      __syncwarp();
    }
    if constexpr (EPI == EPI_BNBWD) {
#pragma unroll
      for (int i = 0; i < 4; ++i) { const int r = i * 8 + sub; stg[r * 4 + (cq ^ ((r >> 1) & 3))] = gz[i]; }
      __syncwarp();
#pragma unroll
      for (int j = 0; j < 4; ++j) az[j] = stg[lane * 4 + (j ^ sx)];
      __syncwarp();
    }
#pragma unroll
    for (int j = 0; j < 8; ++j) { const uint4 t = reinterpret_cast<const uint4*>(srow + c0)[j]; v[4 * j] = t.x; v[4 * j + 1] = t.y; v[4 * j + 2] = t.z; v[4 * j + 3] = t.w; }
    float o[32], s2[32];
    if constexpr (EPI == EPI_BNBWD) {
      const __nv_bfloat162* yb = reinterpret_cast<const __nv_bfloat162*>(ax);
      const __nv_bfloat162* zb = reinterpret_cast<const __nv_bfloat162*>(az);
#define B2G_BNBWD_LOOP(ACTC)                                                                                                   \
  _Pragma("unroll") for (int j = 0; j < 16; ++j) {                                                                             \
    const float2 y2 = __bfloat1622float2(yb[j]), z2 = __bfloat1622float2(zb[j]);                                               \
    o[2 * j] = __uint_as_float(v[2 * j]) * act_grad_from_out(ACTC, y2.x, p.alpha);                                             \
    o[2 * j + 1] = __uint_as_float(v[2 * j + 1]) * act_grad_from_out(ACTC, y2.y, p.alpha);                                     \
    s2[2 * j] = z2.x; s2[2 * j + 1] = z2.y;                                                                                    \
  }
      if (p.act == ACT_LRELU) { B2G_BNBWD_LOOP(ACT_LRELU) }
      else if (p.act == ACT_RELU) { B2G_BNBWD_LOOP(ACT_RELU) }
      else { B2G_BNBWD_LOOP(p.act) }
#undef B2G_BNBWD_LOOP
    } else if constexpr (EPI == EPI_ACTBWD) {
      const __nv_bfloat162* ab = reinterpret_cast<const __nv_bfloat162*>(ax);
#define B2G_ACTBWD_LOOP(ACTC)                                                                                                  \
  _Pragma("unroll") for (int j = 0; j < 16; ++j) {                                                                             \
    const float2 a2 = __bfloat1622float2(ab[j]);                                                                               \
    o[2 * j] = __uint_as_float(v[2 * j]) * act_grad_from_out(ACTC, a2.x, p.alpha);                                             \
    o[2 * j + 1] = __uint_as_float(v[2 * j + 1]) * act_grad_from_out(ACTC, a2.y, p.alpha);                                     \
  }
      if (p.act == ACT_LRELU) { B2G_ACTBWD_LOOP(ACT_LRELU) }
      else if (p.act == ACT_TANH) { B2G_ACTBWD_LOOP(ACT_TANH) }
      else { B2G_ACTBWD_LOOP(p.act) }
#undef B2G_ACTBWD_LOOP
    } else {
#define B2G_EPI_LOOP(ACTC)                                                                                                     \
  _Pragma("unroll") for (int j = 0; j < 32; ++j) {                                                                             \
    float a = __uint_as_float(v[j]);                                                                                           \
    if (AFFINE) a = fmaf(a, p.scale[nb0 + c0 + j], p.bias[nb0 + c0 + j]);                                                      \
    else if (has_bias) a += p.bias[nb0 + c0 + j];                                                                              \
    o[j] = act_fwd(ACTC, a, p.alpha);                                                                                          \
  }
      if (p.act == ACT_IDENTITY) { B2G_EPI_LOOP(ACT_IDENTITY) }
      else if (p.act == ACT_LRELU) { B2G_EPI_LOOP(ACT_LRELU) }
      else if (p.act == ACT_RELU) { B2G_EPI_LOOP(ACT_RELU) }
      else { B2G_EPI_LOOP(p.act) }
#undef B2G_EPI_LOOP
    }
    uint32_t packed[16];
#pragma unroll
    for (int j = 0; j < 16; ++j) {
      __nv_bfloat162 h = __floats2bfloat162_rn(o[2 * j], o[2 * j + 1]);
      packed[j] = *reinterpret_cast<uint32_t*>(&h);
      if constexpr (stats) { const float2 r = __bfloat1622float2(h); o[2 * j] = r.x; o[2 * j + 1] = r.y; }
    }
#pragma unroll
    for (int j = 0; j < 4; ++j) stg[lane * 4 + (j ^ sx)] = make_uint4(packed[4 * j], packed[4 * j + 1], packed[4 * j + 2], packed[4 * j + 3]);
    __syncwarp();
#pragma unroll
    for (int i = 0; i < 4; ++i) { const int r = i * 8 + sub; *reinterpret_cast<uint4*>(p.out + roff_i[i] + c0) = stg[r * 4 + (cq ^ ((r >> 1) & 3))]; }
    __syncwarp();
    if constexpr (stats) {
      if constexpr (EPI == EPI_STATS) {
#pragma unroll
        for (int j = 0; j < 32; ++j) s2[j] = o[j] * o[j];
      } else {
#pragma unroll
        for (int j = 0; j < 32; ++j) s2[j] = o[j] * s2[j];
      }
      warp_colsum32(o, lane); warp_colsum32(s2, lane);
      sst[(q * 2 + 0) * BN + c0 + lane] = o[0];
      sst[(q * 2 + 1) * BN + c0 + lane] = s2[0];
    }
  }
  if constexpr (stats) {
    epi_bar_sync();
    for (int col = ep_tid; col < BN; col += 256) {
#pragma unroll
      for (int st = 0; st < 2; ++st) {
        const float s = ((sst[(0 * 2 + st) * BN + col] + sst[(1 * 2 + st) * BN + col]) + sst[(2 * 2 + st) * BN + col]) + sst[(3 * 2 + st) * BN + col];
        sacc_add(p.acc + (size_t)(group * 2 + st) * 2 * p.OC, (size_t)p.OC, (size_t)(nb0 + col), s);
      }
    }
  }
}

template <int BN>
__device__ __forceinline__ void load_b_tile(const TcConvParams& p, const CUtensorMap* tmB, uint32_t dst, uint32_t bar, int ch, int wtap, int nb0) {
  if (!p.b_mn) tma_load_3d(dst, tmB, bar, ch * 64, wtap, nb0);
  else {
#pragma unroll
    for (int j = 0; j < (BN >= 64 ? BN / 64 : 1); ++j) tma_load_3d(dst + j * 8192, tmB, bar, nb0 + j * 64, wtap, ch * 64);
  }
}
template <int BN, int NB, int NACC>
__device__ __forceinline__ void mma_kblock(float (&acc)[NB][NACC], uint32_t a_smem, uint32_t b_smem, int b_mn) {
  const uint64_t adesc = desc_kmajor_sw128(a_smem);
  if constexpr (BN < 64) {
    const uint64_t bdesc = desc_kmajor_sw128(b_smem);
#pragma unroll
    for (int k = 0; k < 4; ++k) wgmma_n16(acc[0], adesc + 2 * k, bdesc + 2 * k);
  } else if constexpr (NB == 2) {
    if (!b_mn) {
#pragma unroll
      for (int k = 0; k < 4; ++k) wgmma_n128<0, 0>(acc[0], acc[1], adesc + 2 * k, desc_kmajor_sw128(b_smem) + 2 * k);
    } else {
#pragma unroll
      for (int k = 0; k < 4; ++k) wgmma_n128<0, 1>(acc[0], acc[1], adesc + 2 * k, desc_mnmajor_sw128(b_smem + k * 2048, 8192));
    }
  } else if (!b_mn) {
#pragma unroll
    for (int k = 0; k < 4; ++k) wgmma_n64<0, 0>(acc[0], adesc + 2 * k, desc_kmajor_sw128(b_smem) + 2 * k);
  } else {
#pragma unroll
    for (int k = 0; k < 4; ++k) wgmma_n64<0, 1>(acc[0], adesc + 2 * k, desc_mnmajor_sw128(b_smem + k * 2048, 8192));
  }
}
__device__ __forceinline__ void tap_coords(const TcConvParams& p, int ta, int tb, int py, int px, int& ax, int& dy_, int& wtap) {
  if (p.mode == 0) { dy_ = -p.PH + ta; ax = -p.PW + tb; wtap = ta * p.KW + tb; }
  else {
    const int r = py == 0 ? (ta == 0 ? 1 : 3) : (ta == 0 ? 0 : 2), dyr = py == 0 ? (ta == 0 ? 0 : -1) : (ta == 0 ? 1 : 0);
    const int sx = px == 0 ? (tb == 0 ? 1 : 3) : (tb == 0 ? 0 : 2), dxc = px == 0 ? (tb == 0 ? 0 : -1) : (tb == 0 ? 1 : 0);
    dy_ = dyr; ax = dxc; wtap = r * 4 + sx;
  }
}
__device__ __forceinline__ void slab_coords(const TcConvParams& p, int ta, int tb, int py, int px, int& ax, int& dy_, int& wlo, int& whi) {
  int ax2, dy2;
  tap_coords(p, p.mode == 0 ? ta : 1, tb, py, px, ax, dy_, wlo);
  tap_coords(p, p.mode == 0 ? ta + 2 : 0, tb, py, px, ax2, dy2, whi);
}

template <int BN>
struct TcConvRegs {
  static constexpr int LAUNCH = 96, PRODUCER = 24, MMA = BN >= 128 ? 96 : 64, EPI = BN >= 128 ? 128 : 160;
  static_assert(PRODUCER + 2 * MMA + 2 * EPI <= 5 * LAUNCH, "setmaxnreg budget exceeds the launch allocation");
};
template <int BN, int STAGES, int EPI, bool AFFINE, bool PS = false, bool SLAB = false>
__global__ void __launch_bounds__(TC_CONV_THREADS, 1) tc_conv_kernel(const __grid_constant__ CUtensorMap tmA, const __grid_constant__ CUtensorMap tmB, const TcConvParams p) {
  using S = TcSmem<BN, STAGES, EPI, SLAB>;
  using R = TcConvRegs<BN>;
  constexpr int NB = BN >= 64 ? BN / 64 : 1, NACC = BN >= 64 ? 32 : BN / 2;
  extern __shared__ uint8_t smem_raw[];
  const uint32_t smem_base = (smem_u32(smem_raw) + 1023u) & ~1023u;
  uint8_t* smem_gen = smem_raw + (smem_base - smem_u32(smem_raw));
  const uint32_t bar_full = smem_base + S::BAR_OFF;
  const uint32_t bar_empty = bar_full + 8 * STAGES;
  const uint32_t park_full = bar_empty + 8 * STAGES;
  const uint32_t park_empty = park_full + 8 * S::PARKS;
  float* sst = reinterpret_cast<float*>(smem_gen + S::STAT_OFF);
  const int warp = threadIdx.x >> 5, lane = threadIdx.x & 31;
  const int num_kb = p.taps_h * p.taps_w * p.chunks;
  const int tiles = p.tiles_m * p.tiles_n * p.phases;
  auto tile_coords = [&](int t, int& nb0, int& phase, int& n0, int& y0) {
    const int mt = t % p.tiles_m, r = t / p.tiles_m;
    nb0 = (r % p.tiles_n) * BN; phase = r / p.tiles_n;
    if (p.Nt > 1) { n0 = mt * p.Nt; y0 = 0; } else { n0 = mt / p.tiles_y; y0 = (mt % p.tiles_y) * p.Ht; }
  };

  if (threadIdx.x == 0) {
    prefetch_map(&tmA); prefetch_map(&tmB);
    for (int s = 0; s < STAGES; ++s) { mbar_init(bar_full + 8 * s, 1); mbar_init(bar_empty + 8 * s, 8); }
    for (int k = 0; k < S::PARKS; ++k) { mbar_init(park_full + 8 * k, 256); mbar_init(park_empty + 8 * k, 256); }
    fence_mbar_init();
  }
  __syncthreads();
  pdl_wait();

  if (warp >= 16) {
    setmaxnreg_dec<R::PRODUCER>();
    if (warp == 16) {
      int s = 0; uint32_t ph = 0;
      for (int t = blockIdx.x; t < tiles; t += gridDim.x) {
        int nb0, phase, n0, y0; tile_coords(t, nb0, phase, n0, y0);
        const int py = phase >> 1, px = phase & 1;
        const int ybase = p.mode == 0 ? y0 * p.SH : y0;
        int ch = 0, ta = 0, tb = 0;
        int ax, dy_, wtap, wtap2 = 0;
        auto coords = [&]() { if constexpr (SLAB) slab_coords(p, ta, tb, py, px, ax, dy_, wtap, wtap2); else tap_coords(p, ta, tb, py, px, ax, dy_, wtap); };
        coords();
        for (int kb = 0; kb < num_kb; ++kb) {
          mbar_wait(bar_empty + 8 * s, ph ^ 1);
          if (elect_one_sync()) {
            const uint32_t st = smem_base + s * S::STAGE_BYTES;
            mbar_expect_tx(bar_full + 8 * s, SLAB ? p.slab_bytes + S::B_BYTES : S::STAGE_BYTES);
            tma_load_4d(st, &tmA, bar_full + 8 * s, ch * 64, ax, ybase + dy_, n0);
            load_b_tile<BN>(p, &tmB, st + S::A_BYTES, bar_full + 8 * s, ch, wtap, nb0);
            if constexpr (SLAB) load_b_tile<BN>(p, &tmB, st + S::A_BYTES + BN * 128, bar_full + 8 * s, ch, wtap2, nb0);
          }
          __syncwarp();
          if (++s == STAGES) { s = 0; ph ^= 1; }
          if (++ch == p.chunks) { ch = 0; if (++tb == p.taps_w) { tb = 0; ++ta; } coords(); }
        }
      }
    }
  } else if (warp < 8) {
    if constexpr (R::MMA < R::LAUNCH) setmaxnreg_dec<R::MMA>();
    const int wg = warp >> 2;
    const int r0 = wg * 64 + (warp & 3) * 16 + (lane >> 2);
    int s = 0, k = 0; uint32_t ph = 0, kph = 0;
    for (int t = blockIdx.x; t < tiles; t += gridDim.x) {
      float acc[NB][NACC];
#pragma unroll
      for (int nb = 0; nb < NB; ++nb)
#pragma unroll
        for (int j = 0; j < NACC; ++j) acc[nb][j] = 0.f;
      int prev = -1;
      for (int kb = 0; kb < num_kb; ++kb) {
        mbar_wait(bar_full + 8 * s, ph);
        wg_fence();
        const uint32_t st = smem_base + s * S::STAGE_BYTES;
        if constexpr (SLAB) {
          const uint32_t a = st + wg * p.a_wg_bytes;
          mma_kblock<BN, NB, NACC>(acc, a, st + S::A_BYTES, p.b_mn);
          mma_kblock<BN, NB, NACC>(acc, a + p.a_tap_bytes, st + S::A_BYTES + BN * 128, p.b_mn);
        } else {
          mma_kblock<BN, NB, NACC>(acc, st + wg * 8192, st + S::A_BYTES, PS ? 0 : p.b_mn);
        }
        wg_commit();
        wg_wait<1>();
        if (prev >= 0 && lane == 0) mbar_arrive(bar_empty + 8 * prev);
        prev = s;
        if (++s == STAGES) { s = 0; ph ^= 1; }
      }
      wg_wait<0>();
      if (lane == 0) mbar_arrive(bar_empty + 8 * prev);
      mbar_wait(park_empty + 8 * k, kph ^ 1);
      float* park = reinterpret_cast<float*>(smem_gen + S::PARK_OFF + k * S::PARK_BYTES);
#pragma unroll
      for (int nb = 0; nb < NB; ++nb)
#pragma unroll
        for (int j = 0; j < NACC / 4; ++j) {
          const int col = nb * 64 + j * 8 + 2 * (lane & 3);
          *reinterpret_cast<float2*>(park + r0 * S::ACC_PITCH + col) = make_float2(acc[nb][4 * j], acc[nb][4 * j + 1]);
          *reinterpret_cast<float2*>(park + (r0 + 8) * S::ACC_PITCH + col) = make_float2(acc[nb][4 * j + 2], acc[nb][4 * j + 3]);
        }
      mbar_arrive(park_full + 8 * k);
      if (++k == S::PARKS) { k = 0; kph ^= 1; }
    }
  } else {
    setmaxnreg_inc<R::EPI>();
    const int ew = warp - 8, q = ew & 3, half = ew >> 2;
    const int row = q * 32 + lane;
    const int img = row / (p.Ht * p.Wt), rem = row % (p.Ht * p.Wt), yy = rem / p.Wt, xx = rem % p.Wt;
    int k = 0; uint32_t kph = 0;
    for (int t = blockIdx.x; t < tiles; t += gridDim.x) {
      int nb0, phase, n0, y0; tile_coords(t, nb0, phase, n0, y0);
      const int py = phase >> 1, px = phase & 1;
      const int n = n0 + img, gy = y0 + yy, gx = xx;
      mbar_wait(park_full + 8 * k, kph);
      const float* srow = reinterpret_cast<const float*>(smem_gen + S::PARK_OFF + k * S::PARK_BYTES) + row * S::ACC_PITCH;
      if constexpr (PS) {
        if (half == 0) {
          const int C = p.OC;
#pragma unroll
          for (int ppy = 0; ppy < 2; ++ppy) {
            const size_t doff = (((size_t)n * p.outH + 2 * gy + ppy) * p.outW + 2 * gx) * C;
            __nv_bfloat16* dst = p.out + doff;
            float o[8];
#pragma unroll
            for (int ppx = 0; ppx < 2; ++ppx)
#pragma unroll
              for (int c = 0; c < 4; ++c) {
                float a = srow[(ppy * 2 + ppx) * 4 + c];
                if constexpr (EPI == EPI_ACTBWD) { if (c < C) a *= act_grad_from_out(p.act, __bfloat162float(p.aux[doff + ppx * C + c]), p.alpha); }
                else { if (p.bias && c < C) a += p.bias[c]; a = act_fwd(p.act, a, p.alpha); }
                o[ppx * 4 + c] = a;
              }
            if (C == 3) {
              __nv_bfloat162 h0 = __floats2bfloat162_rn(o[0], o[1]), h1 = __floats2bfloat162_rn(o[2], o[4]), h2 = __floats2bfloat162_rn(o[5], o[6]);
              uint32_t* d32 = reinterpret_cast<uint32_t*>(dst);
              d32[0] = *reinterpret_cast<uint32_t*>(&h0); d32[1] = *reinterpret_cast<uint32_t*>(&h1); d32[2] = *reinterpret_cast<uint32_t*>(&h2);
            } else {
#pragma unroll
              for (int ppx = 0; ppx < 2; ++ppx)
#pragma unroll
                for (int c = 0; c < 4; ++c) if (c < C) dst[ppx * C + c] = __float2bfloat16(o[ppx * 4 + c]);
            }
          }
        }
      } else {
        size_t pix;
        if (p.mode == 0) pix = ((size_t)n * p.outH + gy) * p.outW + gx;
        else pix = ((size_t)n * p.outH + 2 * gy + py) * p.outW + 2 * gx + px;
        const int group = p.imgs_per_group > 0 ? n0 / p.imgs_per_group : 0;
        epi_tile<BN, EPI, AFFINE>(p, srow, pix * p.OC + nb0, nb0, group, sst, reinterpret_cast<uint4*>(smem_gen + S::STG_OFF) + ew * 128, q, lane,
                                  (int)threadIdx.x - 256, half * (BN / 2), (half + 1) * (BN / 2));
        if constexpr (EPI == EPI_STATS || EPI == EPI_BNBWD) epi_bar_sync();
      }
      mbar_arrive(park_empty + 8 * k);
      if (++k == S::PARKS) { k = 0; kph ^= 1; }
    }
  }
}

const char* g_tc_last_kernel = "";
bool g_tc_last_slab = false;
int g_tc_test_bn = 0, g_tc_test_max_ctas = 0, g_tc_test_per_tap = 0, g_tc_test_splits = 0;
int g_tc_last_splits = 0;
static int tc_device() { int dev = 0; cudaGetDevice(&dev); return dev < 0 || dev >= 64 ? 0 : dev; }
#define TC_SET_SMEM_ONCE(kernel, bytes)                                                                                            \
  do { static bool set_[64] = {}; const int d_ = tc_device();                                                                       \
       if (!set_[d_]) { if (cudaFuncSetAttribute(kernel, cudaFuncAttributeMaxDynamicSharedMemorySize, (int)(bytes)) != cudaSuccess) return -2; set_[d_] = true; } } while (0)

static bool pick_row_tile(int N, int GH, int GW, int rows, int* Nt, int* Ht, int* Wt) {
  const int P = GH * GW;
  if (GW > rows || rows % GW) return false;
  if (P >= rows) { if (P % rows) return false; *Nt = 1; *Ht = rows / GW; *Wt = GW; return GH % *Ht == 0; }
  if (rows % P || N % (rows / P)) return false;
  *Nt = rows / P; *Ht = GH; *Wt = GW; return true;
}
static int pick_bn(int OC) { return OC % 128 == 0 ? 128 : OC % 64 == 0 ? 64 : 0; }
static int pick_bn_fill(int OC, long m_tiles_x_phases) {
  if (g_tc_test_bn) return g_tc_test_bn;
  const int target = device_sm_count();
  int bn = pick_bn(OC);
  while (bn > 64 && m_tiles_x_phases * (OC / bn) < target) bn /= 2;
  return bn;
}

bool tc_fprop_supported(const ConvGeom& g) {
  int a, b, c;
  return g.C % 64 == 0 && pick_bn(g.O) != 0 && g.SH >= 1 && g.SH <= 2 && g.SW == g.SH && g.KH * g.KW * (g.C / 64) >= 1 &&
         pick_row_tile(g.N, g.OH, g.OW, 128, &a, &b, &c) && c * g.SW <= 256 && b * g.SH <= 256 && g.N >= 1;
}
bool tc_dgrad_supported(const ConvGeom& g) {
  int a, b, c;
  return g.KH == 4 && g.KW == 4 && g.SH == 2 && g.SW == 2 && g.PH == 1 && g.PW == 1 && g.O % 64 == 0 && pick_bn(g.C) != 0 && g.H == 2 * g.OH && g.W == 2 * g.OW &&
         pick_row_tile(g.N, g.OH, g.OW, 128, &a, &b, &c);
}
static bool tc_epi_ok(const TcEpi* e, int Nt) { return !e || e->mode == EPI_PLAIN || e->mode == EPI_ACTBWD || (e->imgs_per_group > 0 && e->imgs_per_group % Nt == 0 && e->acc); }

template <int BN, int STAGES, int EPI, bool AFFINE, bool PS = false, bool SLAB = false>
static int launch_conv_e(const CUtensorMap& tmA, const CUtensorMap& tmB, const TcConvParams& p, cudaStream_t s) {
  using S = TcSmem<BN, STAGES, EPI, SLAB>;
  TC_SET_SMEM_ONCE((tc_conv_kernel<BN, STAGES, EPI, AFFINE, PS, SLAB>), S::TOTAL);
  const long tiles = (long)p.tiles_m * p.tiles_n * p.phases;
  const unsigned grid = (unsigned)std::min<long>(tiles, g_tc_test_max_ctas > 0 ? g_tc_test_max_ctas : device_sm_count());
  launch_pdl(tc_conv_kernel<BN, STAGES, EPI, AFFINE, PS, SLAB>, dim3(grid), dim3(TC_CONV_THREADS), (size_t)(S::TOTAL), s, tmA, tmB, p);
  LAUNCHED();
  return cudaPeekAtLastError() == cudaSuccess ? 0 : -3;
}
template <int BN, int STAGES, bool SLAB>
static int launch_conv(const CUtensorMap& tmA, const CUtensorMap& tmB, const TcConvParams& p, cudaStream_t s, const char* name) {
  g_tc_last_kernel = name; g_tc_last_slab = SLAB;
  switch (p.epi) {
    case EPI_STATS: return launch_conv_e<BN, STAGES, EPI_STATS, false, false, SLAB>(tmA, tmB, p, s);
    case EPI_BNBWD: return launch_conv_e<BN, STAGES, EPI_BNBWD, false, false, SLAB>(tmA, tmB, p, s);
    case EPI_ACTBWD: return launch_conv_e<BN, STAGES, EPI_ACTBWD, false, false, SLAB>(tmA, tmB, p, s);
  }
  return (p.scale && p.bias) ? launch_conv_e<BN, STAGES, EPI_PLAIN, true, false, SLAB>(tmA, tmB, p, s) : launch_conv_e<BN, STAGES, EPI_PLAIN, false, false, SLAB>(tmA, tmB, p, s);
}
static int dispatch_conv(int BN, bool slab, const CUtensorMap& tmA, const CUtensorMap& tmB, const TcConvParams& p, cudaStream_t s) {
  switch (BN * 2 + slab) {
    case 128: return launch_conv<64, 4, false>(tmA, tmB, p, s, "tc_conv_kernel<64,4>");
    case 256: return launch_conv<128, 4, false>(tmA, tmB, p, s, "tc_conv_kernel<128,4>");
    case 129: return launch_conv<64, 4, true>(tmA, tmB, p, s, "tc_conv_kernel<64,4>");
  }
  return -4;
}
static bool slab_tile(const TcConvParams& p, int BN) {
  if (g_tc_test_per_tap || BN != 64 || p.Wt % 8) return false;
  if (!((p.Nt == 1 && p.Ht >= 2) || (p.Nt == 2 && p.Ht * p.Wt == 64))) return false;
  return p.Nt * (p.Ht + 1) * p.Wt <= SLAB_ROWS;
}
static bool is_k4s2p1_geom(const ConvGeom& g) { return g.KH == 4 && g.KW == 4 && g.SH == 2 && g.SW == 2 && g.PH == 1 && g.PW == 1 && g.H == 2 * g.OH && g.W == 2 * g.OW; }
static void set_slab(TcConvParams& p) {
  p.taps_h = p.mode == 0 ? 2 : 1;
  p.slab_bytes = p.Nt * (p.Ht + 1) * p.Wt * 128;
  p.a_wg_bytes = p.Nt == 1 ? 64 * 128 : (p.Ht + 1) * p.Wt * 128;
  p.a_tap_bytes = p.Wt * 128;
}

static int weight_map(CUtensorMap* m, const __nv_bfloat16* w, int rows, int taps, int inner, int box_rows) {
  cuuint64_t dims[3] = {(cuuint64_t)inner, (cuuint64_t)taps, (cuuint64_t)rows};
  cuuint64_t strides[2] = {(cuuint64_t)inner * 2, (cuuint64_t)taps * inner * 2};
  cuuint32_t box[3] = {64, 1, (cuuint32_t)box_rows}; cuuint32_t es[3] = {1, 1, 1};
  return make_map_bf16(m, w, 3, dims, strides, box, es);
}
static void fill_epi(TcConvParams& p, const float* bias, int act, float alpha, const TcEpi* e) {
  p.bias = bias; p.act = act; p.alpha = alpha; p.epi = EPI_PLAIN;
  if (!e) return;
  p.scale = e->scale; p.epi = e->mode; p.acc = e->acc; p.imgs_per_group = e->mode == EPI_STATS || e->mode == EPI_BNBWD ? e->imgs_per_group : 0;
  p.aux = e->aux; p.aux2 = e->aux2;
  if (e->mode == EPI_BNBWD || e->mode == EPI_ACTBWD) { p.act = e->act; p.alpha = e->alpha; p.bias = nullptr; p.scale = nullptr; }
}

int k_tc_fprop(const ConvGeom& g, const __nv_bfloat16* x, const __nv_bfloat16* w, const float* bias, __nv_bfloat16* out, int act, float alpha, cudaStream_t s, const TcEpi* epi, int w_mn) {
  TcConvParams p{}; p.mode = 0;
  if (!pick_row_tile(g.N, g.OH, g.OW, 128, &p.Nt, &p.Ht, &p.Wt) || !tc_epi_ok(epi, p.Nt)) return -1;
  if (w_mn && (g.KH != 1 || g.KW != 1)) return -1;
  const int BN = pick_bn_fill(g.O, (long)g.N * g.OH * g.OW / 128);
  p.GH = g.OH; p.GW = g.OW; p.tiles_y = g.OH / p.Ht; p.taps_h = g.KH; p.taps_w = g.KW; p.chunks = g.C / 64; p.KW = g.KW;
  p.SH = g.SH; p.SW = g.SW; p.PH = g.PH; p.PW = g.PW; p.OC = g.O; p.outH = g.OH; p.outW = g.OW; p.out = out; p.b_mn = w_mn;
  fill_epi(p, bias, act, alpha, epi);
  const bool slab = is_k4s2p1_geom(g) && !w_mn && slab_tile(p, BN);
  if (slab) set_slab(p);
  CUtensorMap tmA, tmB;
  cuuint64_t dims[4] = {(cuuint64_t)g.C, (cuuint64_t)g.W, (cuuint64_t)g.H, (cuuint64_t)g.N};
  cuuint64_t strides[3] = {(cuuint64_t)g.C * 2, (cuuint64_t)g.W * g.C * 2, (cuuint64_t)g.H * g.W * g.C * 2};
  cuuint32_t box[4] = {64, (cuuint32_t)(p.Wt * g.SW), (cuuint32_t)((p.Ht + slab) * g.SH), (cuuint32_t)p.Nt};
  cuuint32_t es[4] = {1, (cuuint32_t)g.SW, (cuuint32_t)g.SH, 1};
  if (make_map_bf16(&tmA, x, 4, dims, strides, box, es)) return -1;
  p.tiles_m = g.N * g.OH * g.OW / 128; p.tiles_n = g.O / BN; p.phases = 1;
  if (w_mn ? weight_map(&tmB, w, g.C, 1, g.O, 64) : weight_map(&tmB, w, g.O, g.KH * g.KW, g.C, BN)) return -1;
  return dispatch_conv(BN, slab, tmA, tmB, p, s);
}

int k_tc_dgrad(const ConvGeom& g, const __nv_bfloat16* dy, const __nv_bfloat16* w, const float* bias, __nv_bfloat16* dx, int act, float alpha, cudaStream_t s, const TcEpi* epi) {
  TcConvParams p{}; p.mode = 1;
  if (!pick_row_tile(g.N, g.OH, g.OW, 128, &p.Nt, &p.Ht, &p.Wt) || !tc_epi_ok(epi, p.Nt)) return -1;
  const int BN = pick_bn_fill(g.C, (long)g.N * g.OH * g.OW / 128 * 4);
  p.GH = g.OH; p.GW = g.OW; p.tiles_y = g.OH / p.Ht; p.taps_h = 2; p.taps_w = 2; p.chunks = g.O / 64; p.KW = 4;
  p.SH = 1; p.SW = 1; p.PH = 0; p.PW = 0; p.OC = g.C; p.outH = g.H; p.outW = g.W; p.out = dx; p.b_mn = 1;
  fill_epi(p, bias, act, alpha, epi);
  const bool slab = slab_tile(p, BN);
  if (slab) set_slab(p);
  CUtensorMap tmA, tmB;
  cuuint64_t dims[4] = {(cuuint64_t)g.O, (cuuint64_t)g.OW, (cuuint64_t)g.OH, (cuuint64_t)g.N};
  cuuint64_t strides[3] = {(cuuint64_t)g.O * 2, (cuuint64_t)g.OW * g.O * 2, (cuuint64_t)g.OH * g.OW * g.O * 2};
  cuuint32_t box[4] = {64, (cuuint32_t)p.Wt, (cuuint32_t)(p.Ht + slab), (cuuint32_t)p.Nt};
  cuuint32_t es[4] = {1, 1, 1, 1};
  if (weight_map(&tmB, w, g.O, 16, g.C, 64)) return -1;
  if (make_map_bf16(&tmA, dy, 4, dims, strides, box, es)) return -1;
  p.tiles_m = g.N * g.OH * g.OW / 128; p.tiles_n = g.C / BN; p.phases = 4;
  return dispatch_conv(BN, slab, tmA, tmB, p, s);
}

bool tc_deconv_ps_shape(const ConvGeom& g) { return is_k4s2p1_geom(g) && g.C >= 1 && g.C <= 4 && g.O % 64 == 0; }
bool tc_deconv_ps_supported(const ConvGeom& g) { int a, b, c; return tc_deconv_ps_shape(g) && pick_row_tile(g.N, g.OH, g.OW, 128, &a, &b, &c); }
size_t k_tc_deconv_ps_weight_elems(const ConvGeom& g) { return tc_deconv_ps_shape(g) ? (size_t)16 * 9 * g.O : 0; }
__global__ void pack_deconv_ps_kernel(const float* __restrict__ w, __nv_bfloat16* __restrict__ wps, int O, int C) { pdl_wait();
  const int idx = blockIdx.x * blockDim.x + threadIdx.x; if (idx >= 16 * 9 * O) return;
  const int o = idx % O, t = (idx / O) % 9, n = idx / (9 * O);
  const int py = n >> 3, px = (n >> 2) & 1, c = n & 3, dyr = t / 3 - 1, dxc = t % 3 - 1;
  const int r = dyr == -1 ? (py == 0 ? 3 : -1) : dyr == 0 ? (py == 0 ? 1 : 2) : (py == 1 ? 0 : -1);
  const int sx = dxc == -1 ? (px == 0 ? 3 : -1) : dxc == 0 ? (px == 0 ? 1 : 2) : (px == 1 ? 0 : -1);
  wps[idx] = __float2bfloat16((r >= 0 && sx >= 0 && c < C) ? w[((size_t)o * 16 + r * 4 + sx) * C + c] : 0.f);
}
void k_pack_deconv_ps(const float* w, __nv_bfloat16* wps, int O, int C, cudaStream_t s) {
  launch_pdl(pack_deconv_ps_kernel, dim3((16 * 9 * O + 255) / 256), dim3(256), (size_t)(0), s, w, wps, O, C); LAUNCHED();
}
int k_tc_deconv_ps(const ConvGeom& g, const __nv_bfloat16* dy, const __nv_bfloat16* wps, const float* bias, __nv_bfloat16* dx, int act, float alpha, cudaStream_t s, const TcEpi* epi) {
  TcConvParams p{}; p.mode = 0;
  if (!tc_deconv_ps_shape(g) || !pick_row_tile(g.N, g.OH, g.OW, 128, &p.Nt, &p.Ht, &p.Wt)) return -1;
  if (epi && epi->mode != EPI_PLAIN && epi->mode != EPI_ACTBWD) return -1;
  p.GH = g.OH; p.GW = g.OW; p.tiles_y = g.OH / p.Ht; p.taps_h = 3; p.taps_w = 3; p.chunks = g.O / 64; p.KW = 3;
  p.SH = 1; p.SW = 1; p.PH = 1; p.PW = 1; p.OC = g.C; p.outH = g.H; p.outW = g.W; p.out = dx;
  fill_epi(p, bias, act, alpha, epi);
  CUtensorMap tmA, tmB;
  cuuint64_t dims[4] = {(cuuint64_t)g.O, (cuuint64_t)g.OW, (cuuint64_t)g.OH, (cuuint64_t)g.N};
  cuuint64_t strides[3] = {(cuuint64_t)g.O * 2, (cuuint64_t)g.OW * g.O * 2, (cuuint64_t)g.OH * g.OW * g.O * 2};
  cuuint32_t box[4] = {64, (cuuint32_t)p.Wt, (cuuint32_t)p.Ht, (cuuint32_t)p.Nt}; cuuint32_t es[4] = {1, 1, 1, 1};
  if (make_map_bf16(&tmA, dy, 4, dims, strides, box, es)) return -1;
  if (weight_map(&tmB, wps, 16, 9, g.O, 16)) return -1;
  p.tiles_m = (int)((long)g.N * g.OH * g.OW / 128); p.tiles_n = 1; p.phases = 1;
  g_tc_last_kernel = "tc_conv_kernel<16,4,PS>";
  return p.epi == EPI_ACTBWD ? launch_conv_e<16, 4, EPI_ACTBWD, false, true>(tmA, tmB, p, s) : launch_conv_e<16, 4, EPI_PLAIN, false, true>(tmA, tmB, p, s);
}

struct TcEdgeParams {
  const __nv_bfloat16* x; const __nv_bfloat16* w; const __nv_bfloat16* dy; const float* bias; __nv_bfloat16* out; float* part; float* part_b;
  int N, H, W, C, OH, OW, O, Ht, tiles_y, tiles_total, tiles_per_cta, act; float alpha;
};
static constexpr int EDGE_SLAB_BYTES = 6144;
__device__ __forceinline__ uint32_t swz128(int row, int byte) { return (uint32_t)(row * 128 + ((((byte >> 4) ^ (row & 7)) << 4) | (byte & 15))); }

struct EdgeSlabRegs { uint4 v[3]; };
__device__ __forceinline__ void edge_fetch_slab(const TcEdgeParams& p, int n, int oy0, EdgeSlabRegs& r) {
  const int WC = p.W * p.C, cpr = WC >> 3, total = (2 * p.Ht + 2) * cpr;
#pragma unroll
  for (int q = 0; q < 3; ++q) {
    const int i = threadIdx.x + q * 128; r.v[q] = make_uint4(0u, 0u, 0u, 0u);
    if (i < total) { const int j = i / cpr, cc = i - j * cpr, iy = 2 * oy0 - 1 + j;
      if (iy >= 0 && iy < p.H) r.v[q] = __ldg(reinterpret_cast<const uint4*>(p.x + ((size_t)n * p.H + iy) * WC) + cc); }
  }
}
__device__ __forceinline__ void edge_store_slab(const TcEdgeParams& p, const EdgeSlabRegs& r, uint8_t* slab) {
  const int total = (2 * p.Ht + 2) * ((p.W * p.C) >> 3);
#pragma unroll
  for (int q = 0; q < 3; ++q) { const int i = threadIdx.x + q * 128; if (i < total) reinterpret_cast<uint4*>(slab)[i] = r.v[q]; }
}
template <int C>
__device__ __forceinline__ void edge_build_row_c(const TcEdgeParams& p, const uint8_t* slab, uint8_t* tile, int row, bool ones) {
  const int WC = p.W * C, oy_l = row / p.OW, ox = row - oy_l * p.OW;
  const int lo = ox == 0 ? C : 0, hi = ox == p.OW - 1 ? 3 * C : 4 * C;
  uint32_t out[32];
#pragma unroll
  for (int i = 0; i < 32; ++i) out[i] = 0u;
#pragma unroll
  for (int r = 0; r < 4; ++r) {
    const int b0 = ((2 * oy_l + r) * WC + (2 * ox - 1) * C) * 2;
    if (C & 1) {
      const uint32_t* wp = reinterpret_cast<const uint32_t*>(slab + b0 - 2);
      uint32_t w[2 * C + 1];
#pragma unroll
      for (int i = 0; i <= 2 * C; ++i) w[i] = wp[i];
#pragma unroll
      for (int i = 0; i < 2 * C; ++i) out[r * 2 * C + i] = __funnelshift_r(w[i], w[i + 1], 16);
    } else {
      const uint32_t* wp = reinterpret_cast<const uint32_t*>(slab + b0);
#pragma unroll
      for (int i = 0; i < 2 * C; ++i) out[r * 2 * C + i] = wp[i];
    }
#pragma unroll
    for (int i = 0; i < 2 * C; ++i) {
      const uint32_t m = ((2 * i >= lo && 2 * i < hi) ? 0xFFFFu : 0u) | ((2 * i + 1 >= lo && 2 * i + 1 < hi) ? 0xFFFF0000u : 0u);
      out[r * 2 * C + i] &= m;
    }
  }
  if (C < 4 && ones) out[8 * C] = 0x3F80u;
#pragma unroll
  for (int cc = 0; cc < 8; ++cc) *reinterpret_cast<uint4*>(tile + row * 128 + ((cc ^ (row & 7)) << 4)) = make_uint4(out[4 * cc], out[4 * cc + 1], out[4 * cc + 2], out[4 * cc + 3]);
}
__device__ __forceinline__ void edge_build_row(const TcEdgeParams& p, const uint8_t* slab, uint8_t* tile, int row, bool ones = false) {
  switch (p.C) { case 1: edge_build_row_c<1>(p, slab, tile, row, ones); break; case 2: edge_build_row_c<2>(p, slab, tile, row, ones); break;
                 case 3: edge_build_row_c<3>(p, slab, tile, row, ones); break; default: edge_build_row_c<4>(p, slab, tile, row, ones); break; }
}


__global__ void __launch_bounds__(128) tc_edge_conv_kernel(const TcEdgeParams p) { pdl_wait();
  extern __shared__ uint8_t smem_raw[];
  const uint32_t smem_base = (smem_u32(smem_raw) + 1023u) & ~1023u;
  uint8_t* sm = smem_raw + (smem_base - smem_u32(smem_raw));
  uint8_t* sA = sm; uint8_t* sB = sm + 16384; uint8_t* slab = sm + 24576;
  const int tid = threadIdx.x, warp = tid >> 5, lane = tid & 31;
  const int nb0 = blockIdx.y * 64, K = 16 * p.C;
  const int t_beg = blockIdx.x * p.tiles_per_cta, t_end = min(p.tiles_total, t_beg + p.tiles_per_cta);
  EdgeSlabRegs pre;
  if (t_beg < t_end) edge_fetch_slab(p, t_beg / p.tiles_y, (t_beg % p.tiles_y) * p.Ht, pre);
  {
    uint4 wv[4];
#pragma unroll
    for (int q = 0; q < 4; ++q) { const int i = tid + q * 128, o = i >> 3, cc = i & 7;
      wv[q] = cc < 2 * p.C ? __ldg(reinterpret_cast<const uint4*>(p.w + (size_t)(nb0 + o) * K) + cc) : make_uint4(0u, 0u, 0u, 0u); }
#pragma unroll
    for (int q = 0; q < 4; ++q) { const int i = tid + q * 128, o = i >> 3, cc = i & 7; *reinterpret_cast<uint4*>(sB + o * 128 + ((cc ^ (o & 7)) << 4)) = wv[q]; }
  }
  const bool has_bias = p.bias != nullptr;
  const int r0 = warp * 16 + (lane >> 2), cq = lane & 3;
  for (int t = t_beg; t < t_end; ++t) {
    const int n = t / p.tiles_y, oy0 = (t % p.tiles_y) * p.Ht;
    edge_store_slab(p, pre, slab);
    __syncthreads();
    if (t + 1 < t_end) edge_fetch_slab(p, (t + 1) / p.tiles_y, ((t + 1) % p.tiles_y) * p.Ht, pre);
    edge_build_row(p, slab, sA, tid);
    fence_proxy_async_smem();
    __syncthreads();
    float acc[2][32];
#pragma unroll
    for (int h = 0; h < 2; ++h)
#pragma unroll
      for (int j = 0; j < 32; ++j) acc[h][j] = 0.f;
    wg_fence();
    {
      const uint64_t bdesc = desc_kmajor_sw128(smem_base + 16384);
#pragma unroll
      for (int k = 0; k < 4; ++k)
#pragma unroll
        for (int h = 0; h < 2; ++h) wgmma_n64<0, 0>(acc[h], desc_kmajor_sw128(smem_base + h * 8192) + 2 * k, bdesc + 2 * k);
    }
    wg_commit();
    wg_wait<0>();
    __syncthreads();
#pragma unroll
    for (int h = 0; h < 2; ++h)
#pragma unroll
      for (int i = 0; i < 2; ++i) {
        const int row = h * 64 + r0 + 8 * i;
#pragma unroll
        for (int j = 0; j < 8; ++j) {
          const int col = j * 8 + 2 * cq;
          float a = acc[h][4 * j + 2 * i], b = acc[h][4 * j + 2 * i + 1];
          if (has_bias) { a += p.bias[nb0 + col]; b += p.bias[nb0 + col + 1]; }
          __nv_bfloat162 v = __floats2bfloat162_rn(act_fwd(p.act, a, p.alpha), act_fwd(p.act, b, p.alpha));
          *reinterpret_cast<__nv_bfloat162*>(sA + row * 128 + ((j ^ (row & 7)) << 4) + cq * 4) = v;
        }
      }
    __syncthreads();
// ... 263 lines not shown
```

gan_deeplearning4j_b200/engine.py:

```python
from __future__ import annotations

import copy
import ctypes as C
import math
from typing import Dict, List, Optional, Sequence

import numpy as np

from . import _lib
from ._lib import GanConfig, LayerDesc, LrSchedule, NetConfig, check

LAYER_TYPES = {"conv2d": 0, "deconv2d": 1, "batchnorm": 2, "dense": 3, "activation": 4, "maxpool": 5, "upsample2d": 6,
               "output": 7, "loss": 8, "ff_to_cnn": 9, "cnn_to_ff": 10, "dropout": 11, "subsampling": 12, "global_pooling": 13}
POOLINGS = {"max": 0, "avg": 1, "sum": 2, "pnorm": 3}
GLOBAL_PNORM_DEFAULT = 2
ACTS = {"identity": 0, "tanh": 1, "sigmoid": 2, "relu": 3, "lrelu": 4, "elu": 5, "selu": 6, "softplus": 7, "softsign": 8, "hardtanh": 9,
        "hardsigmoid": 10, "relu6": 11, "swish": 12, "cube": 13, "rationaltanh": 14, "rectifiedtanh": 15, "thresholdedrelu": 16}
ACT_ALPHA_DEFAULTS = {"elu": 1.0, "thresholdedrelu": 1.0}
LOSSES = {"xent": 0, "mcxent": 1, "mse": 2, "l1": 3, "l2": 4, "mae": 5, "hinge": 6, "squared_hinge": 7, "wasserstein": 8}
UPDATERS = {"sgd": 0, "rmsprop": 1, "adam": 2, "noop": 3, "nesterovs": 4, "adagrad": 5, "adamax": 6, "nadam": 7, "amsgrad": 8, "adadelta": 9}
NO_LR_UPDATERS = ("noop", "adadelta")
GRADIENT_NORMALIZATIONS = {"none": 0, "renormalize_l2_per_layer": 1, "renormalize_l2_per_param_type": 2, "clip_l2_per_layer": 4,
                           "clip_l2_per_param_type": 5}
SCHEDULE_KINDS = {"exponential": 1, "inverse": 2, "sigmoid": 3, "step": 4, "map": 5}
# ... 265 lines not shown

    def compute_gradient_and_score(self, x, y) -> float:
        x, y = _f32(x), _f32(y)
        s = C.c_float()
        check(self.lib.b2g_net_compute_gradient_and_score(self.h, _fp(x), _fp(y), x.shape[0], C.byref(s)))
        return s.value

    def fit(self, x, y) -> float:
        x, y = _f32(x), _f32(y)
        s = C.c_float()
        check(self.lib.b2g_net_fit(self.h, _fp(x), _fp(y), x.shape[0], C.byref(s)))
        return s.value

    def set_gradient_normalization(self, mode: str, threshold: float = 1.0):
        if mode not in GRADIENT_NORMALIZATIONS:
            raise ValueError(f"unknown gradient normalization {mode!r}; one of {sorted(GRADIENT_NORMALIZATIONS)} (element-wise clipping is grad_clip)")
        check(self.lib.b2g_net_set_gradient_normalization(self.h, GRADIENT_NORMALIZATIONS[mode], float(threshold)))

    def set_lr_schedule(self, schedule: Optional[Dict], layer: Optional[str] = None):
        s, _arrays = schedule_struct(schedule)
        check(self.lib.b2g_net_set_lr_schedule(self.h, None if layer is None else layer.encode(), C.byref(s)))
        follow_lr_schedule(self.specs, self.lr_constants, schedule, layer)

    def learning_rate(self, layer: str) -> float:
        v = C.c_float()
        check(self.lib.b2g_net_get_learning_rate(self.h, layer.encode(), C.byref(v)))
        return v.value

    def epoch(self) -> int:
        v = C.c_int64()
        check(self.lib.b2g_net_get_epoch(self.h, C.byref(v)))
        return v.value

    def set_epoch(self, epoch: int):
        check(self.lib.b2g_net_set_epoch(self.h, int(epoch)))

    def set_grad_allreduce(self, enabled: bool):
        check(self.lib.b2g_net_set_grad_allreduce(self.h, int(enabled)))

    def set_sync_bn(self, enabled: bool):
        check(self.lib.b2g_net_set_sync_bn(self.h, int(enabled)))

    def set_grad_payload_bf16(self, enabled: bool):
        check(self.lib.b2g_net_set_grad_payload_bf16(self.h, int(enabled)))

    def enable_p2p_allreduce(self) -> bool:
        out = C.c_int32(0)
        check(self.lib.b2g_net_enable_p2p_allreduce(self.h, C.byref(out)))
        return bool(out.value)

    def average_parameters(self):
        check(self.lib.b2g_net_average_parameters(self.h))

    def iteration(self) -> int:
        v = C.c_int64()
        check(self.lib.b2g_net_get_iteration(self.h, C.byref(v)))
        return v.value

    def set_iteration(self, it: int):
        check(self.lib.b2g_net_set_iteration(self.h, int(it)))

    def dropout_pass(self) -> int:
        v = C.c_int64()
        check(self.lib.b2g_net_get_dropout_pass(self.h, C.byref(v)))
        return v.value

    def set_dropout_pass(self, p: int):
        check(self.lib.b2g_net_set_dropout_pass(self.h, int(p)))

    def simt_gemm_calls(self) -> int:
        v = C.c_uint64()
        check(self.lib.b2g_net_simt_gemm_calls(self.h, C.byref(v)))
        return v.value

    def time_hbm_kernels(self, rows: int, channels: int, iters: int = 10):
        ms = np.zeros(3, np.float32)
        check(self.lib.b2g_test_hbm_kernels(self.h, rows, channels, iters, _fp(ms)))
        return [float(v) for v in ms]

    def weight_operand(self, layer: int, which: int, size: int) -> np.ndarray:
        out = np.empty(size, np.float32)
        check(self.lib.b2g_test_net_shadow(self.h, layer, which, _fp(out), out.size))
        return out

    def input_gradient(self, batch: int) -> np.ndarray:
        out = np.empty((batch, int(np.prod(self.input_shape))), np.float32)
        check(self.lib.b2g_net_get_input_gradient(self.h, batch, _fp(out)))
        return out

    def close(self):
        if self.h:
            self.lib.b2g_net_destroy(self.h)
            self.h = None


class Gan:

    def __init__(self, gen: Net, dis: Net, fake_bn_train: bool = False, use_cuda_graph: bool = True):
        self.gen, self.dis, self.lib = gen, dis, gen.lib
        cfg = GanConfig(int(fake_bn_train), int(use_cuda_graph))
        h = C.c_void_p()
        check(self.lib.b2g_gan_create(gen.h, dis.h, C.byref(cfg), C.byref(h)))
        self.h = h

    def step(self, x_real, z_d, z_g, y_real, y_fake, y_gen):
        a = [_f32(v) for v in (x_real, z_d, z_g, y_real, y_fake, y_gen)]
        losses = np.zeros(3, np.float32)
        check(self.lib.b2g_gan_step(self.h, *[_fp(v) for v in a], a[0].shape[0], _fp(losses)))
        return losses

    def step_ptr(self, ptrs, batch: int, losses: np.ndarray):
        args = [C.cast(C.c_void_p(p), C.POINTER(C.c_float)) for p in ptrs]
        check(self.lib.b2g_gan_step(self.h, *args, batch, _fp(losses)))

    def upload(self, x_real, z_d, z_g, y_real, y_fake, y_gen):
        a = [_f32(v) for v in (x_real, z_d, z_g, y_real, y_fake, y_gen)]
        check(self.lib.b2g_gan_upload(self.h, *[_fp(v) for v in a], a[0].shape[0]))
        self.gen.ctx.sync()

    def step_resident(self, batch: int):
        check(self.lib.b2g_gan_step_resident(self.h, batch))

    def losses(self) -> np.ndarray:
        out = np.zeros(3, np.float32)
        check(self.lib.b2g_gan_read_losses(self.h, _fp(out)))
        return out

    def last_step_ms(self) -> float:
        v = C.c_float()
        check(self.lib.b2g_gan_last_step_ms(self.h, C.byref(v)))
        return v.value

    def close(self):
        if self.h:
            self.lib.b2g_gan_destroy(self.h)
            self.h = None


def test_conv(ctx: Context, kind: int, impl: int, precision: int, geom: Dict[str, int], a, b, out_size: int, iters: int = 1):
    g = _lib.ConvGeom(**geom)
    a, b = _f32(a).ravel(), _f32(b).ravel()
    out = np.empty(out_size, np.float32)
    ms = C.c_float()
    check(ctx.lib.b2g_test_conv(ctx.h, kind, impl, precision, C.byref(g), _fp(a), _fp(b), _fp(out), iters, C.byref(ms)))
    return out, ms.value


EPI_PLAIN, EPI_STATS, EPI_BNBWD, EPI_ACTBWD = 0, 1, 2, 3


def test_conv_ex(ctx: Context, kind: int, geom: Dict[str, int], a, b, out_size: int, *, epi: int = 0, act: str = "identity", alpha: float = 0.0,
                 bias=None, scale=None, groups: int = 1, aux=None, aux2=None, iters: int = 1, impl: int = 1, bn: int = 0, max_ctas: int = 0,
                 poison: bool = False, w_mn: bool = False, per_tap: bool = False, info: Optional[dict] = None, defer: bool = False, db=None,
                 precision: int = BF16, param_offset: int = 0, splits: int = 0):
    g = _lib.ConvGeom(**geom)
    a, b = _f32(a).ravel(), _f32(b).ravel()
    out = np.empty(out_size, np.float32)
    oc = geom["o"] if kind == 0 else geom["c"]
    o = _lib.TestConvOpts()
    o.epi, o.act, o.alpha, o.groups = epi, ACTS[act], alpha, groups
    o.bn, o.max_ctas, o.poison, o.w_mn, o.per_tap, o.defer = bn, max_ctas, int(poison), int(w_mn), int(per_tap), int(defer)
    o.param_offset, o.splits = param_offset, splits
    if db is not None:
        assert db.dtype == np.float32 and db.flags.c_contiguous
        o.db = _fp(db)
    keep = []
    for name, v in (("bias", bias), ("scale", scale), ("aux", aux), ("aux2", aux2)):
        if v is not None:
            arr = _f32(v).ravel(); keep.append(arr); setattr(o, name, _fp(arr))
    stats = None
    if epi in (EPI_STATS, EPI_BNBWD):
        stats = np.zeros((groups, 2, oc), np.float64); o.stats = stats.ctypes.data_as(C.POINTER(C.c_double))
    ms = C.c_float()
    check(ctx.lib.b2g_test_conv_ex(ctx.h, kind, impl, precision, C.byref(g), _fp(a), _fp(b), _fp(out), iters, C.byref(ms), C.byref(o)))
    if info is not None:
        info["slab"], info["splits"] = bool(o.slab), o.splits
    return out, stats, o.kernel.decode(), ms.value


def test_bn(ctx: Context, precision: int, path: int, x, eps_out, gamma, beta, run_mean, run_var, *, act: str = "identity", alpha: float = 0.0,
            eps: float = 1e-5, decay: float = 0.9, g_gamma=None, g_beta=None, want_param_grads: bool = True):
    x, e = _f32(x), _f32(eps_out)
    groups, rows, ch = x.shape
    par = [_f32(v).ravel() for v in (gamma, beta, run_mean, run_var)]
    r = {k: np.empty(x.shape, np.float32) for k in ("y", "eps_in")}
    r["g_gamma"] = _f32(np.zeros(ch) if g_gamma is None else g_gamma).copy()
    r["g_beta"] = _f32(np.zeros(ch) if g_beta is None else g_beta).copy()
    r.update({k: np.empty(ch, np.float32) for k in ("g_mean", "g_var")})
    r.update({k: np.empty((groups, ch), np.float32) for k in ("mean", "invstd")})
    check(ctx.lib.b2g_test_bn(ctx.h, precision, path, groups, rows, ch, _fp(x), _fp(e), *[_fp(v) for v in par], ACTS[act], alpha, eps, decay,
                              int(want_param_grads), *[_fp(r[k]) for k in ("y", "eps_in", "g_gamma", "g_beta", "g_mean", "g_var", "mean", "invstd")]))
    return r


def test_dropout(ctx: Context, precision: int, x, dy, p: float, *, seed: int = 666, layer: int = 0, rank: int = 0, pass_: int = 0):
    x, e = _f32(x), _f32(dy)
    rows = x.shape[0]
    h, w, c = (x.shape[1:] if x.ndim == 4 else (1, 1, int(np.prod(x.shape[1:]))))
    y, dx = np.empty_like(x), np.empty_like(x)
    check(ctx.lib.b2g_test_dropout(ctx.h, precision, seed, layer, rank, pass_, rows, h, w, c, p, _fp(x), _fp(e), _fp(y), _fp(dx)))
    return y, dx


EW_OPS = {"reduce_splits": 0, "reduce_multi": 1, "colsum": 2, "xent": 3, "softmax_xent": 4, "act_fwd": 5, "act_bwd": 6, "maxpool": 7,
          "upsample": 8, "sumsq": 9, "loss": 10, "act_ext_fwd": 11, "act_ext_bwd": 12}


def test_ew(ctx: Context, precision: int, op: str, in0, in1=None, out_sizes=(0, 0, 0), *, act: str = "identity", jobs=None, segments=None,
            loss: str = "xent", **opts):
    o = _lib.TestEwOpts()
    o.op, o.act, o.loss = EW_OPS[op], ACTS[act], LOSSES[loss]
    for k, v in opts.items():
        setattr(o, k, int(v) if isinstance(v, bool) else v)
    keep = []
    if jobs is not None:
        arr = (_lib.EwReduceJob * len(jobs))(*[_lib.EwReduceJob(j["n"], j["stride"], j["src_off"], j["dst_off"], j["splits"], 0) for j in jobs])
        o.n_jobs, o.jobs = len(jobs), arr
        keep.append(arr)
    if segments is not None:
        so, sl, sc = (np.ascontiguousarray(segments[0], np.int64), np.ascontiguousarray(segments[1], np.int64), _f32(segments[2]))
        keep += [so, sl, sc]
        o.n_seg = len(so)
        o.seg_off, o.seg_len, o.seg_coef = so.ctypes.data_as(C.POINTER(C.c_int64)), sl.ctypes.data_as(C.POINTER(C.c_int64)), _fp(sc)
    ins = [None if v is None else _f32(v).ravel() for v in (in0, in1)]
    outs = [np.empty(k, np.float32) if k else None for k in out_sizes]
    ptr = lambda a: None if a is None else _fp(a)
    check(ctx.lib.b2g_test_ew(ctx.h, precision, C.byref(o), *[ptr(a) for a in ins], *[ptr(a) for a in outs]))
    info = {"kernel": o.kernel.decode(), "sumsq": o.sumsq, "wide": [o.jobs[i].wide for i in range(o.n_jobs)] if jobs is not None else []}
    return outs, info


POOL_TEST_OPS = {"pool2d": 0, "global_pool": 1}


def test_pool(ctx: Context, precision: int, op: str, in0, in1, out_sizes=(0, 0, 0), *, pooling: str = "max", pnorm: float = 2.0, **opts):
    o = _lib.TestPoolOpts()
    o.op, o.pool, o.pnorm = POOL_TEST_OPS[op], POOLINGS[pooling], float(pnorm)
    for k, v in opts.items():
        setattr(o, k, int(v))
    ins = [_f32(v).ravel() for v in (in0, in1)]
    outs = [np.empty(k, np.float32) if k else None for k in out_sizes]
    ptr = lambda a: None if a is None else _fp(a)
    check(ctx.lib.b2g_test_pool(ctx.h, precision, C.byref(o), *[ptr(a) for a in ins], *[ptr(a) for a in outs]))
    return outs, {"kernel": o.kernel.decode(), "splits": o.splits}
```

include/b200gan.h:

```cpp
#ifndef B200GAN_H
#define B200GAN_H

#include <stddef.h>
#include <stdint.h>

#ifdef __cplusplus
extern "C" {
#endif

#define B2G_VERSION 101
#define B2G_NAME_LEN 64

typedef struct b2g_ctx b2g_ctx;
typedef struct b2g_net b2g_net;
typedef struct b2g_gan b2g_gan;

typedef enum {
  B2G_OK = 0,
  B2G_ERR_ARG = -1,
  B2G_ERR_SHAPE = -2,
  B2G_ERR_CUDA = -3,
  B2G_ERR_NCCL = -4,
  B2G_ERR_OOM = -5,
  B2G_ERR_UNSUPPORTED = -6,
// ... 17 lines not shown
  B2G_LAYER_GLOBAL_POOLING = 13
} b2g_layer_type;


typedef enum { B2G_POOL_MAX = 0, B2G_POOL_AVG = 1, B2G_POOL_SUM = 2, B2G_POOL_PNORM = 3 } b2g_pooling;

typedef enum {
  B2G_ACT_IDENTITY = 0, B2G_ACT_TANH = 1, B2G_ACT_SIGMOID = 2, B2G_ACT_RELU = 3, B2G_ACT_LRELU = 4,
  B2G_ACT_ELU = 5, B2G_ACT_SELU = 6, B2G_ACT_SOFTPLUS = 7, B2G_ACT_SOFTSIGN = 8, B2G_ACT_HARDTANH = 9, B2G_ACT_HARDSIGMOID = 10,
  B2G_ACT_RELU6 = 11, B2G_ACT_SWISH = 12, B2G_ACT_CUBE = 13, B2G_ACT_RATIONALTANH = 14, B2G_ACT_RECTIFIEDTANH = 15, B2G_ACT_THRESHOLDEDRELU = 16
} b2g_activation;

typedef enum {
  B2G_UPD_SGD = 0, B2G_UPD_RMSPROP = 1, B2G_UPD_ADAM = 2, B2G_UPD_NOOP = 3, B2G_UPD_NESTEROVS = 4, B2G_UPD_ADAGRAD = 5, B2G_UPD_ADAMAX = 6,
  B2G_UPD_NADAM = 7, B2G_UPD_AMSGRAD = 8, B2G_UPD_ADADELTA = 9
} b2g_updater;

typedef enum { B2G_PREC_FP32 = 0, B2G_PREC_BF16 = 1 } b2g_precision;
typedef enum {
  B2G_LOSS_XENT = 0, B2G_LOSS_MCXENT = 1, B2G_LOSS_MSE = 2, B2G_LOSS_L1 = 3, B2G_LOSS_L2 = 4, B2G_LOSS_MAE = 5, B2G_LOSS_HINGE = 6,
  B2G_LOSS_SQUARED_HINGE = 7, B2G_LOSS_WASSERSTEIN = 8
} b2g_loss;

typedef struct {
  int32_t type;
  char name[B2G_NAME_LEN];
  int32_t n_in, n_out;
  int32_t k_h, k_w, s_h, s_w, p_h, p_w;
  int32_t has_bias;
  int32_t act;
  float act_alpha;
  int32_t updater;
  float lr, beta1, beta2, eps;
  float l2;
  float bn_decay, bn_eps;
  int32_t pre_h, pre_w, pre_c;
  int32_t loss;
  int32_t frozen;
} b2g_layer_desc;

typedef struct {
  int32_t in_h, in_w, in_c;
  int32_t max_batch;
  int32_t precision;
  float grad_clip;
  float xent_clip_eps;
  int32_t bn_groups;
  uint64_t seed;
} b2g_net_config;

int32_t b2g_version(void);
int32_t b2g_ctx_create(int32_t device, b2g_ctx** out);
int32_t b2g_ctx_destroy(b2g_ctx* ctx);
const char* b2g_last_error(void);
int32_t b2g_sync(b2g_ctx* ctx);
int32_t b2g_launch_count(b2g_ctx* ctx, uint64_t* out);
int32_t b2g_timer_start(b2g_ctx* ctx);
int32_t b2g_timer_stop_ms(b2g_ctx* ctx, float* ms);
int32_t b2g_flush_l2(b2g_ctx* ctx);
int32_t b2g_device_info(b2g_ctx* ctx, int32_t* sm_count, int32_t* cc_major, int32_t* cc_minor, uint64_t* mem_bytes);

int32_t b2g_net_create(b2g_ctx* ctx, const b2g_net_config* cfg, const b2g_layer_desc* layers, int32_t n_layers, b2g_net** out);
int32_t b2g_net_destroy(b2g_net* net);
int32_t b2g_net_num_params(b2g_net* net, int64_t* out);
int32_t b2g_net_output_size(b2g_net* net, int64_t* per_example);
int32_t b2g_net_layer_output_size(b2g_net* net, int32_t layer, int64_t* per_example);
int32_t b2g_net_set_param(b2g_net* net, const char* layer, const char* param, const float* host, int64_t n);
int32_t b2g_net_get_param(b2g_net* net, const char* layer, const char* param, float* host, int64_t n);
int32_t b2g_net_get_params(b2g_net* net, float* host, int64_t n);
int32_t b2g_net_set_params(b2g_net* net, const float* host, int64_t n);
int32_t b2g_net_get_gradients(b2g_net* net, float* host, int64_t n);
int32_t b2g_net_updater_state_size(b2g_net* net, int64_t* out);
int32_t b2g_net_get_updater_state(b2g_net* net, float* host, int64_t n);
int32_t b2g_net_set_updater_state(b2g_net* net, const float* host, int64_t n);
int32_t b2g_net_output(b2g_net* net, const float* x, int32_t batch, int32_t train, float* out);
int32_t b2g_net_get_activation(b2g_net* net, int32_t layer, int32_t batch, float* host);
int32_t b2g_net_compute_gradient_and_score(b2g_net* net, const float* x, const float* y, int32_t batch, float* score);
int32_t b2g_net_get_input_gradient(b2g_net* net, int32_t batch, float* host);
int32_t b2g_net_fit(b2g_net* net, const float* x, const float* y, int32_t batch, float* score);
int32_t b2g_net_get_iteration(b2g_net* net, int64_t* out);
int32_t b2g_net_set_iteration(b2g_net* net, int64_t iteration);
int32_t b2g_net_get_dropout_pass(b2g_net* net, int64_t* out);
int32_t b2g_net_set_dropout_pass(b2g_net* net, int64_t pass);
typedef enum {
  B2G_GN_NONE = 0, B2G_GN_RENORM_L2_LAYER = 1, B2G_GN_RENORM_L2_PARAM = 2, B2G_GN_CLIP_ELEMENTWISE = 3, B2G_GN_CLIP_L2_LAYER = 4, B2G_GN_CLIP_L2_PARAM = 5
} b2g_gradient_normalization;
int32_t b2g_net_set_gradient_normalization(b2g_net* net, int32_t mode, float threshold);
typedef enum {
  B2G_SCHED_NONE = 0, B2G_SCHED_EXPONENTIAL = 1, B2G_SCHED_INVERSE = 2, B2G_SCHED_SIGMOID = 3, B2G_SCHED_STEP = 4, B2G_SCHED_MAP = 5
} b2g_schedule_kind;
typedef enum { B2G_SCHED_ITERATION = 0, B2G_SCHED_EPOCH = 1 } b2g_schedule_type;
typedef struct {
  int32_t kind, type;
  double initial, gamma, power, step, decay_rate;
  int32_t n_map;
  const int32_t* map_keys;
  const double* map_values;
} b2g_lr_schedule;
int32_t b2g_net_set_lr_schedule(b2g_net* net, const char* layer, const b2g_lr_schedule* s);
int32_t b2g_net_get_learning_rate(b2g_net* net, const char* layer, float* out);
int32_t b2g_net_get_epoch(b2g_net* net, int64_t* out);
int32_t b2g_net_set_epoch(b2g_net* net, int64_t epoch);
int32_t b2g_net_simt_gemm_calls(b2g_net* net, uint64_t* out);

typedef struct {
  int32_t fake_bn_train;
  int32_t use_cuda_graph;
} b2g_gan_config;
int32_t b2g_gan_create(b2g_net* gen, b2g_net* dis, const b2g_gan_config* cfg, b2g_gan** out);
int32_t b2g_gan_destroy(b2g_gan* gan);
int32_t b2g_gan_step(b2g_gan* gan, const float* x_real, const float* z_d, const float* z_g,
                     const float* y_real, const float* y_fake, const float* y_gen, int32_t batch, float* losses);
int32_t b2g_gan_upload(b2g_gan* gan, const float* x_real, const float* z_d, const float* z_g,
                       const float* y_real, const float* y_fake, const float* y_gen, int32_t batch);
int32_t b2g_gan_step_resident(b2g_gan* gan, int32_t batch);
int32_t b2g_gan_read_losses(b2g_gan* gan, float* losses);
int32_t b2g_gan_last_step_ms(b2g_gan* gan, float* ms);

#define B2G_NCCL_ID_BYTES 128
int32_t b2g_comm_unique_id(void* id128);
int32_t b2g_ctx_comm_init(b2g_ctx* ctx, int32_t world, int32_t rank, const void* id128);
int32_t b2g_ctx_comm_destroy(b2g_ctx* ctx);
int32_t b2g_net_set_grad_allreduce(b2g_net* net, int32_t enabled);
int32_t b2g_net_average_parameters(b2g_net* net);
int32_t b2g_net_set_sync_bn(b2g_net* net, int32_t enabled);
int32_t b2g_net_set_grad_payload_bf16(b2g_net* net, int32_t enabled);
int32_t b2g_net_enable_p2p_allreduce(b2g_net* net, int32_t* enabled);
int32_t b2g_ctx_allreduce_test(b2g_ctx* ctx, float* host_inout, int64_t n);

typedef struct {
  int32_t n, h, w, c;
  int32_t oh, ow, o;
  int32_t kh, kw, sh, sw, ph, pw;
} b2g_conv_geom;
int32_t b2g_test_conv(b2g_ctx* ctx, int32_t kind, int32_t impl, int32_t precision, const b2g_conv_geom* g,
                      const float* x_or_dy, const float* w_or_x, float* out, int32_t iters, float* ms_per_iter);
typedef struct {
  int32_t epi;
  int32_t act; float alpha;
  const float* bias;
  const float* scale;
  int32_t groups;
  const float* aux;
  const float* aux2;
  double* stats;
  char kernel[64];
  int32_t bn;
  int32_t max_ctas;
  int32_t poison;
  int32_t w_mn;
  int32_t per_tap;
  int32_t slab;
  int32_t defer;
  float* db;
  int32_t param_offset;
  int32_t splits;
} b2g_test_conv_opts;
int32_t b2g_test_conv_ex(b2g_ctx* ctx, int32_t kind, int32_t impl, int32_t precision, const b2g_conv_geom* g,
                         const float* x_or_dy, const float* w_or_x, float* out, int32_t iters, float* ms_per_iter, b2g_test_conv_opts* opts);

int32_t b2g_test_hbm_kernels(b2g_net* net, int32_t rows, int32_t channels, int32_t iters, float* ms3);

int32_t b2g_test_bn(b2g_ctx* ctx, int32_t precision, int32_t path, int32_t groups, int32_t rows, int32_t C, const float* x, const float* eps_out,
                    const float* gamma, const float* beta, const float* run_mean, const float* run_var, int32_t act, float alpha, float eps, float decay,
                    int32_t want_param_grads, float* y, float* eps_in, float* g_gamma, float* g_beta, float* g_mean, float* g_var, float* mean, float* invstd);
int32_t b2g_test_net_shadow(b2g_net* net, int32_t layer, int32_t which, float* out, int64_t n);
int32_t b2g_test_dropout(b2g_ctx* ctx, int32_t precision, uint64_t seed, int32_t layer, int32_t rank, int64_t pass, int32_t rows, int32_t h, int32_t w,
                         int32_t c, float p, const float* x, const float* dy, float* y, float* dx);

typedef enum {
  B2G_EW_REDUCE_SPLITS = 0, B2G_EW_REDUCE_MULTI = 1, B2G_EW_COLSUM = 2, B2G_EW_XENT = 3, B2G_EW_SOFTMAX_XENT = 4,
  B2G_EW_ACT_FWD = 5, B2G_EW_ACT_BWD = 6, B2G_EW_MAXPOOL = 7, B2G_EW_UPSAMPLE = 8, B2G_EW_SUMSQ = 9, B2G_EW_LOSS = 10,
  B2G_EW_ACT_EXT_FWD = 11, B2G_EW_ACT_EXT_BWD = 12
} b2g_ew_op;
typedef struct {
  int64_t n, stride, src_off, dst_off;
  int32_t splits;
  int32_t wide;
} b2g_ew_reduce_job;
typedef struct {
  int32_t op;
  int64_t n;
  int32_t rows, cols;
  int32_t groups;
  int32_t splits; int64_t stride;
  int32_t N, H, W, C, KH, KW, SH, SW;
  int32_t act; float alpha;
  float clip_eps;
  int32_t offset;
  int32_t in_place;
  int32_t accumulate;
  int32_t poison;
  int32_t n_jobs; b2g_ew_reduce_job* jobs;
  int32_t n_seg; const int64_t* seg_off; const int64_t* seg_len; const float* seg_coef;
  double sumsq;
  char kernel[64];
  int32_t loss;
} b2g_test_ew_opts;
int32_t b2g_test_ew(b2g_ctx* ctx, int32_t precision, b2g_test_ew_opts* opts, const float* in0, const float* in1, float* out0, float* out1, float* out2);

typedef enum { B2G_TEST_POOL2D = 0, B2G_TEST_GLOBAL_POOL = 1 } b2g_test_pool_op;
typedef struct {
  int32_t op;
  int32_t pool;
  float pnorm;
  int32_t N, H, W, C, KH, KW, SH, SW, PH, PW;
  int32_t offset;
  int32_t poison;
  char kernel[64];
  int32_t splits;
} b2g_test_pool_opts;
int32_t b2g_test_pool(b2g_ctx* ctx, int32_t precision, b2g_test_pool_opts* opts, const float* in0, const float* in1, float* out0, float* out1, float* out2);

#ifdef __cplusplus
}
#endif
#endif
```

Before: 92350.

## Keep dgrad weight tiles resident in shared memory across M tiles

Adds a RESB variant of the tensor-core conv kernel for BN=64 dgrad. When all weight k-blocks fit in 64 KB, they stay resident in shared memory, and each CTA handles a contiguous range of tiles instead of a strided one. Weights are then reloaded only when the N-tile/phase key changes, which cuts repeated TMA loads of B and frees ring bandwidth. The cost is extra mbarrier bookkeeping, more shared memory that shrinks the park area budget, and a contiguous tile split that may balance load less evenly across CTAs.

Result: no change. 92290, median of 6 (-0.1%).

```diff
diff --git a/gan_deeplearning4j_b200/_lib.py b/gan_deeplearning4j_b200/_lib.py
--- a/gan_deeplearning4j_b200/_lib.py
+++ b/gan_deeplearning4j_b200/_lib.py
@@ -46,7 +46,7 @@
     _fields_ = [("epi", C.c_int32), ("act", C.c_int32), ("alpha", C.c_float), ("bias", C.POINTER(C.c_float)), ("scale", C.POINTER(C.c_float)),
                 ("groups", C.c_int32), ("aux", C.POINTER(C.c_float)), ("aux2", C.POINTER(C.c_float)), ("stats", C.POINTER(C.c_double)), ("kernel", C.c_char * 64),
                 ("bn", C.c_int32), ("max_ctas", C.c_int32), ("poison", C.c_int32), ("w_mn", C.c_int32), ("per_tap", C.c_int32), ("slab", C.c_int32),
-                ("defer", C.c_int32), ("db", C.POINTER(C.c_float)), ("param_offset", C.c_int32), ("splits", C.c_int32)]
+                ("defer", C.c_int32), ("resb", C.c_int32), ("db", C.POINTER(C.c_float)), ("param_offset", C.c_int32), ("splits", C.c_int32)]
 
 
 class EwReduceJob(C.Structure):
diff --git a/gan_deeplearning4j_b200/csrc/engine.cu b/gan_deeplearning4j_b200/csrc/engine.cu
--- a/gan_deeplearning4j_b200/csrc/engine.cu
+++ b/gan_deeplearning4j_b200/csrc/engine.cu
@@ -1378,9 +1378,11 @@
 }
 
 struct TcTestSchedule {
-  TcTestSchedule(int bn, int max_ctas, int per_tap, int splits) { g_tc_test_bn = bn; g_tc_test_max_ctas = max_ctas; g_tc_test_per_tap = per_tap; g_tc_test_splits = splits; }
+  TcTestSchedule(int bn, int max_ctas, int per_tap, int splits, int no_resb) {
+    g_tc_test_bn = bn; g_tc_test_max_ctas = max_ctas; g_tc_test_per_tap = per_tap; g_tc_test_splits = splits; g_tc_test_no_resb = no_resb;
+  }
   ~TcTestSchedule() { reset(); }
-  void reset() { g_tc_test_bn = 0; g_tc_test_max_ctas = 0; g_tc_test_per_tap = 0; g_tc_test_splits = 0; }
+  void reset() { g_tc_test_bn = 0; g_tc_test_max_ctas = 0; g_tc_test_per_tap = 0; g_tc_test_splits = 0; g_tc_test_no_resb = 0; }
 };
 extern "C" int32_t b2g_test_conv_ex(b2g_ctx* c, int32_t kind, int32_t impl, int32_t precision, const b2g_conv_geom* gg, const float* a_host, const float* b_host, float* out, int32_t iters, float* ms_per_iter,
                                     b2g_test_conv_opts* opt) {
@@ -1415,6 +1417,8 @@
   const int force_bn = opt ? opt->bn : 0, max_ctas = opt ? opt->max_ctas : 0;
   const bool poison = opt && opt->poison, w_mn = opt && opt->w_mn, per_tap = opt && opt->per_tap;
   if (per_tap && !tc_conv) return fail(B2G_ERR_UNSUPPORTED, "per_tap applies to the tensor-core fprop / dgrad kernels (impl 1, kind 0 / 1)");
+  const int resb_in = opt ? opt->resb : 0;
+  if (resb_in != 0 && (resb_in != -1 || !tc_conv)) return fail(B2G_ERR_UNSUPPORTED, "resb %d: -1 keeps the weights of a tensor-core fprop / dgrad (impl 1, kind 0 / 1) on the ring, 0 is the production choice", resb_in);
   if (force_bn && (!tc_conv || (force_bn != 64 && force_bn != 128) || oc % force_bn))
     return fail(B2G_ERR_UNSUPPORTED, "bn %d: the tensor-core fprop / dgrad tile is 64 or 128 columns and must divide the %d output channels", force_bn, oc);
   if (max_ctas < 0 || (max_ctas && !tc_conv && !ps && !edge_fwd))
@@ -1472,8 +1476,8 @@
   }
   cudaEvent_t e0, e1; CU(cudaEventCreate(&e0)); CU(cudaEventCreate(&e1));
   int reps = iters < 1 ? 1 : iters; int rc = 0;
-  g_tc_last_kernel = ""; g_tc_last_slab = false; g_tc_last_splits = 0; g_gemm_last_kernel = ""; g_gemm_last_splits = 0;
-  TcTestSchedule schedule(force_bn, max_ctas, per_tap, force_splits);
+  g_tc_last_kernel = ""; g_tc_last_slab = false; g_tc_last_resb = false; g_tc_last_splits = 0; g_gemm_last_kernel = ""; g_gemm_last_splits = 0;
+  TcTestSchedule schedule(force_bn, max_ctas, per_tap, force_splits, resb_in == -1);
   for (int it = -1; it < reps; ++it) {
     if (it == 0) CU(cudaEventRecord(e0, s));
     if (d_acc) CU(cudaMemsetAsync(d_acc, 0, 8 * k_bn_acc_elems(oc, groups), s));
@@ -1509,6 +1513,7 @@
   if (rc) return fail(B2G_ERR_CUDA, "tensor-core kernel launch failed (%d)", rc);
   if (opt) {
     strncpy(opt->kernel, gemm ? g_gemm_last_kernel : g_tc_last_kernel, sizeof(opt->kernel) - 1); opt->kernel[sizeof(opt->kernel) - 1] = 0; opt->slab = g_tc_last_slab;
+    opt->resb = g_tc_last_resb;
     opt->splits = gemm ? g_gemm_last_splits : tc_wg ? g_tc_last_splits : 0;
   }
   if (d_db) {
diff --git a/gan_deeplearning4j_b200/csrc/kernels.h b/gan_deeplearning4j_b200/csrc/kernels.h
--- a/gan_deeplearning4j_b200/csrc/kernels.h
+++ b/gan_deeplearning4j_b200/csrc/kernels.h
@@ -154,6 +154,8 @@
 extern int g_tc_test_bn, g_tc_test_max_ctas;
 extern int g_tc_test_per_tap;
 extern bool g_tc_last_slab;
+extern int g_tc_test_no_resb;
+extern bool g_tc_last_resb;
 extern int g_tc_test_splits, g_tc_last_splits;
 enum { EPI_PLAIN = 0, EPI_STATS = 1, EPI_BNBWD = 2, EPI_ACTBWD = 3 };
 struct TcEpi {
diff --git a/gan_deeplearning4j_b200/csrc/kernels_tc.cu b/gan_deeplearning4j_b200/csrc/kernels_tc.cu
--- a/gan_deeplearning4j_b200/csrc/kernels_tc.cu
+++ b/gan_deeplearning4j_b200/csrc/kernels_tc.cu
@@ -129,18 +129,23 @@
 static constexpr int TC_THREADS = 384;
 static constexpr int TC_CONV_THREADS = 640;
 static constexpr int SLAB_ROWS = 144;
-template <int BN, int STAGES, int EPI = EPI_PLAIN, bool SLAB = false>
+static constexpr int RESB_BYTES = 64 * 1024;
+static constexpr int RESB_UNITS = 8;
+template <int BN, int STAGES, int EPI = EPI_PLAIN, bool SLAB = false, bool RESB = false>
 struct TcSmem {
   static constexpr int A_BYTES = (SLAB ? SLAB_ROWS : 128) * 128;
-  static constexpr int B_BYTES = (SLAB ? 2 : 1) * BN * 128;
+  static constexpr int B_UNIT = (SLAB ? 2 : 1) * BN * 128;
+  static constexpr int B_BYTES = RESB ? 0 : B_UNIT;
   static constexpr int STAGE_BYTES = A_BYTES + B_BYTES;
   static constexpr int RING_BYTES = STAGES * STAGE_BYTES;
+  static constexpr int RESB_OFF = RING_BYTES;
   static constexpr int ACC_PITCH = BN + 4;
   static constexpr int PARK_BYTES = 128 * ACC_PITCH * 4;
   static constexpr int PARKS = BN >= 128 ? 1 : 2;
-  static constexpr int PARK_OFF = RING_BYTES;
+  static constexpr int PARK_OFF = RING_BYTES + (RESB ? RESB_BYTES : 0);
   static constexpr int BAR_OFF = PARK_OFF + PARKS * PARK_BYTES;
   static constexpr int STAT_OFF = BAR_OFF + 256;
+  static_assert(16 * STAGES + 16 * PARKS + (RESB ? 16 * RESB_UNITS : 0) <= 256, "the mbarriers must fit their 256-byte area");
   static constexpr int STG_OFF = STAT_OFF + ((EPI == EPI_STATS || EPI == EPI_BNBWD) ? 4 * 2 * BN * 4 : 0);
   static constexpr int TOTAL = STG_OFF + (BN >= 32 ? 8 * 2048 : 0) + 1024;
   static_assert(TOTAL <= 227 * 1024, "one CTA per SM must fit the shared memory of an sm_90 SM");
@@ -331,9 +336,12 @@
   static constexpr int LAUNCH = 96, PRODUCER = 24, MMA = BN >= 128 ? 96 : 64, EPI = BN >= 128 ? 128 : 160;
   static_assert(PRODUCER + 2 * MMA + 2 * EPI <= 5 * LAUNCH, "setmaxnreg budget exceeds the launch allocation");
 };
-template <int BN, int STAGES, int EPI, bool AFFINE, bool PS = false, bool SLAB = false>
+template <bool RESB> __device__ __forceinline__ int tile_first(int tiles) { return RESB ? (int)((long long)blockIdx.x * tiles / gridDim.x) : (int)blockIdx.x; }
+template <bool RESB> __device__ __forceinline__ int tile_end(int tiles) { return RESB ? (int)((long long)(blockIdx.x + 1) * tiles / gridDim.x) : tiles; }
+template <bool RESB> __device__ __forceinline__ unsigned tile_step() { return RESB ? 1u : gridDim.x; }
+template <int BN, int STAGES, int EPI, bool AFFINE, bool PS = false, bool SLAB = false, bool RESB = false>
 __global__ void __launch_bounds__(TC_CONV_THREADS, 1) tc_conv_kernel(const __grid_constant__ CUtensorMap tmA, const __grid_constant__ CUtensorMap tmB, const TcConvParams p) {
-  using S = TcSmem<BN, STAGES, EPI, SLAB>;
+  using S = TcSmem<BN, STAGES, EPI, SLAB, RESB>;
   using R = TcConvRegs<BN>;
   constexpr int NB = BN >= 64 ? BN / 64 : 1, NACC = BN >= 64 ? 32 : BN / 2;
   extern __shared__ uint8_t smem_raw[];
@@ -343,6 +351,8 @@
   const uint32_t bar_empty = bar_full + 8 * STAGES;
   const uint32_t park_full = bar_empty + 8 * STAGES;
   const uint32_t park_empty = park_full + 8 * S::PARKS;
+  const uint32_t b_full = park_empty + 8 * S::PARKS;
+  const uint32_t b_empty = b_full + 8 * RESB_UNITS;
   float* sst = reinterpret_cast<float*>(smem_gen + S::STAT_OFF);
   const int warp = threadIdx.x >> 5, lane = threadIdx.x & 31;
   const int num_kb = p.taps_h * p.taps_w * p.chunks;
@@ -357,6 +367,7 @@
     prefetch_map(&tmA); prefetch_map(&tmB);
     for (int s = 0; s < STAGES; ++s) { mbar_init(bar_full + 8 * s, 1); mbar_init(bar_empty + 8 * s, 8); }
     for (int k = 0; k < S::PARKS; ++k) { mbar_init(park_full + 8 * k, 256); mbar_init(park_empty + 8 * k, 256); }
+    if constexpr (RESB) for (int u = 0; u < RESB_UNITS; ++u) { mbar_init(b_full + 8 * u, 1); mbar_init(b_empty + 8 * u, 8); }
     fence_mbar_init();
   }
   __syncthreads();
@@ -366,27 +377,47 @@
     setmaxnreg_dec<R::PRODUCER>();
     if (warp == 16) {
       int s = 0; uint32_t ph = 0;
-      for (int t = blockIdx.x; t < tiles; t += gridDim.x) {
+      int bkey = -1; uint32_t bph = 0;
+      for (int t = tile_first<RESB>(tiles); t < tile_end<RESB>(tiles); t += tile_step<RESB>()) {
         int nb0, phase, n0, y0; tile_coords(t, nb0, phase, n0, y0);
         const int py = phase >> 1, px = phase & 1;
         const int ybase = p.mode == 0 ? y0 * p.SH : y0;
         int ch = 0, ta = 0, tb = 0;
         int ax, dy_, wtap, wtap2 = 0;
         auto coords = [&]() { if constexpr (SLAB) slab_coords(p, ta, tb, py, px, ax, dy_, wtap, wtap2); else tap_coords(p, ta, tb, py, px, ax, dy_, wtap); };
+        bool new_set = false;
+        if constexpr (RESB) { const int key = t / p.tiles_m; new_set = key != bkey; bkey = key; }
         coords();
         for (int kb = 0; kb < num_kb; ++kb) {
           mbar_wait(bar_empty + 8 * s, ph ^ 1);
           if (elect_one_sync()) {
             const uint32_t st = smem_base + s * S::STAGE_BYTES;
-            mbar_expect_tx(bar_full + 8 * s, SLAB ? p.slab_bytes + S::B_BYTES : S::STAGE_BYTES);
-            tma_load_4d(st, &tmA, bar_full + 8 * s, ch * 64, ax, ybase + dy_, n0);
-            load_b_tile<BN>(p, &tmB, st + S::A_BYTES, bar_full + 8 * s, ch, wtap, nb0);
-            if constexpr (SLAB) load_b_tile<BN>(p, &tmB, st + S::A_BYTES + BN * 128, bar_full + 8 * s, ch, wtap2, nb0);
+            if constexpr (RESB) {
+              mbar_expect_tx(bar_full + 8 * s, SLAB ? p.slab_bytes : S::STAGE_BYTES);
+              tma_load_4d(st, &tmA, bar_full + 8 * s, ch * 64, ax, ybase + dy_, n0);
+            } else {
+              mbar_expect_tx(bar_full + 8 * s, SLAB ? p.slab_bytes + S::B_BYTES : S::STAGE_BYTES);
+              tma_load_4d(st, &tmA, bar_full + 8 * s, ch * 64, ax, ybase + dy_, n0);
+              load_b_tile<BN>(p, &tmB, st + S::A_BYTES, bar_full + 8 * s, ch, wtap, nb0);
+              if constexpr (SLAB) load_b_tile<BN>(p, &tmB, st + S::A_BYTES + BN * 128, bar_full + 8 * s, ch, wtap2, nb0);
+            }
+          }
+          if constexpr (RESB) {
+            if (new_set) {
+              mbar_wait(b_empty + 8 * kb, bph ^ 1);
+              if (elect_one_sync()) {
+                const uint32_t dst = smem_base + S::RESB_OFF + kb * S::B_UNIT;
+                mbar_expect_tx(b_full + 8 * kb, S::B_UNIT);
+                load_b_tile<BN>(p, &tmB, dst, b_full + 8 * kb, ch, wtap, nb0);
+                if constexpr (SLAB) load_b_tile<BN>(p, &tmB, dst + BN * 128, b_full + 8 * kb, ch, wtap2, nb0);
+              }
+            }
           }
           __syncwarp();
           if (++s == STAGES) { s = 0; ph ^= 1; }
           if (++ch == p.chunks) { ch = 0; if (++tb == p.taps_w) { tb = 0; ++ta; } coords(); }
         }
+        if constexpr (RESB) { if (new_set) bph ^= 1; }
       }
     }
   } else if (warp < 8) {
@@ -394,7 +425,14 @@
     const int wg = warp >> 2;
     const int r0 = wg * 64 + (warp & 3) * 16 + (lane >> 2);
     int s = 0, k = 0; uint32_t ph = 0, kph = 0;
-    for (int t = blockIdx.x; t < tiles; t += gridDim.x) {
+    int bkey = -1; uint32_t bph = 0;
+    for (int t = tile_first<RESB>(tiles); t < tile_end<RESB>(tiles); t += tile_step<RESB>()) {
+      bool first_of_set = false, last_of_set = false;
+      if constexpr (RESB) {
+        const int key = t / p.tiles_m;
+        first_of_set = key != bkey; bkey = key;
+        last_of_set = t + 1 < tile_end<RESB>(tiles) && (t + 1) / p.tiles_m != key;
+      }
       float acc[NB][NACC];
 #pragma unroll
       for (int nb = 0; nb < NB; ++nb)
@@ -403,23 +441,30 @@
       int prev = -1;
       for (int kb = 0; kb < num_kb; ++kb) {
         mbar_wait(bar_full + 8 * s, ph);
+        if constexpr (RESB) { if (first_of_set) mbar_wait(b_full + 8 * kb, bph); }
         wg_fence();
         const uint32_t st = smem_base + s * S::STAGE_BYTES;
+        auto bt = [&](int off) -> uint32_t { if constexpr (RESB) return smem_base + S::RESB_OFF + kb * S::B_UNIT + off; else return st + S::A_BYTES + off; };
         if constexpr (SLAB) {
           const uint32_t a = st + wg * p.a_wg_bytes;
-          mma_kblock<BN, NB, NACC>(acc, a, st + S::A_BYTES, p.b_mn);
-          mma_kblock<BN, NB, NACC>(acc, a + p.a_tap_bytes, st + S::A_BYTES + BN * 128, p.b_mn);
+          mma_kblock<BN, NB, NACC>(acc, a, bt(0), p.b_mn);
+          mma_kblock<BN, NB, NACC>(acc, a + p.a_tap_bytes, bt(BN * 128), p.b_mn);
         } else {
-          mma_kblock<BN, NB, NACC>(acc, st + wg * 8192, st + S::A_BYTES, PS ? 0 : p.b_mn);
+          mma_kblock<BN, NB, NACC>(acc, st + wg * 8192, bt(0), PS ? 0 : p.b_mn);
         }
         wg_commit();
         wg_wait<1>();
         if (prev >= 0 && lane == 0) mbar_arrive(bar_empty + 8 * prev);
+        if constexpr (RESB) { if (last_of_set && kb > 0 && lane == 0) mbar_arrive(b_empty + 8 * (kb - 1)); }
         prev = s;
         if (++s == STAGES) { s = 0; ph ^= 1; }
       }
       wg_wait<0>();
       if (lane == 0) mbar_arrive(bar_empty + 8 * prev);
+      if constexpr (RESB) {
+        if (last_of_set && lane == 0) mbar_arrive(b_empty + 8 * (num_kb - 1));
+        if (first_of_set) bph ^= 1;
+      }
       mbar_wait(park_empty + 8 * k, kph ^ 1);
       float* park = reinterpret_cast<float*>(smem_gen + S::PARK_OFF + k * S::PARK_BYTES);
 #pragma unroll
@@ -439,7 +484,7 @@
     const int row = q * 32 + lane;
     const int img = row / (p.Ht * p.Wt), rem = row % (p.Ht * p.Wt), yy = rem / p.Wt, xx = rem % p.Wt;
     int k = 0; uint32_t kph = 0;
-    for (int t = blockIdx.x; t < tiles; t += gridDim.x) {
+    for (int t = tile_first<RESB>(tiles); t < tile_end<RESB>(tiles); t += tile_step<RESB>()) {
       int nb0, phase, n0, y0; tile_coords(t, nb0, phase, n0, y0);
       const int py = phase >> 1, px = phase & 1;
       const int n = n0 + img, gy = y0 + yy, gx = xx;
@@ -491,7 +536,9 @@
 
 const char* g_tc_last_kernel = "";
 bool g_tc_last_slab = false;
+bool g_tc_last_resb = false;
 int g_tc_test_bn = 0, g_tc_test_max_ctas = 0, g_tc_test_per_tap = 0, g_tc_test_splits = 0;
+int g_tc_test_no_resb = 0;
 int g_tc_last_splits = 0;
 static int tc_device() { int dev = 0; cudaGetDevice(&dev); return dev < 0 || dev >= 64 ? 0 : dev; }
 #define TC_SET_SMEM_ONCE(kernel, bytes)                                                                                            \
@@ -526,33 +573,41 @@
 }
 static bool tc_epi_ok(const TcEpi* e, int Nt) { return !e || e->mode == EPI_PLAIN || e->mode == EPI_ACTBWD || (e->imgs_per_group > 0 && e->imgs_per_group % Nt == 0 && e->acc); }
 
-template <int BN, int STAGES, int EPI, bool AFFINE, bool PS = false, bool SLAB = false>
+template <int BN, int STAGES, int EPI, bool AFFINE, bool PS = false, bool SLAB = false, bool RESB = false>
 static int launch_conv_e(const CUtensorMap& tmA, const CUtensorMap& tmB, const TcConvParams& p, cudaStream_t s) {
-  using S = TcSmem<BN, STAGES, EPI, SLAB>;
-  TC_SET_SMEM_ONCE((tc_conv_kernel<BN, STAGES, EPI, AFFINE, PS, SLAB>), S::TOTAL);
+  using S = TcSmem<BN, STAGES, EPI, SLAB, RESB>;
+  TC_SET_SMEM_ONCE((tc_conv_kernel<BN, STAGES, EPI, AFFINE, PS, SLAB, RESB>), S::TOTAL);
   const long tiles = (long)p.tiles_m * p.tiles_n * p.phases;
   const unsigned grid = (unsigned)std::min<long>(tiles, g_tc_test_max_ctas > 0 ? g_tc_test_max_ctas : device_sm_count());
-  launch_pdl(tc_conv_kernel<BN, STAGES, EPI, AFFINE, PS, SLAB>, dim3(grid), dim3(TC_CONV_THREADS), (size_t)(S::TOTAL), s, tmA, tmB, p);
+  launch_pdl(tc_conv_kernel<BN, STAGES, EPI, AFFINE, PS, SLAB, RESB>, dim3(grid), dim3(TC_CONV_THREADS), (size_t)(S::TOTAL), s, tmA, tmB, p);
   LAUNCHED();
   return cudaPeekAtLastError() == cudaSuccess ? 0 : -3;
 }
-template <int BN, int STAGES, bool SLAB>
+template <int BN, int STAGES, bool SLAB, bool RESB = false>
 static int launch_conv(const CUtensorMap& tmA, const CUtensorMap& tmB, const TcConvParams& p, cudaStream_t s, const char* name) {
-  g_tc_last_kernel = name; g_tc_last_slab = SLAB;
+  g_tc_last_kernel = name; g_tc_last_slab = SLAB; g_tc_last_resb = RESB;
   switch (p.epi) {
-    case EPI_STATS: return launch_conv_e<BN, STAGES, EPI_STATS, false, false, SLAB>(tmA, tmB, p, s);
-    case EPI_BNBWD: return launch_conv_e<BN, STAGES, EPI_BNBWD, false, false, SLAB>(tmA, tmB, p, s);
-    case EPI_ACTBWD: return launch_conv_e<BN, STAGES, EPI_ACTBWD, false, false, SLAB>(tmA, tmB, p, s);
-  }
-  return (p.scale && p.bias) ? launch_conv_e<BN, STAGES, EPI_PLAIN, true, false, SLAB>(tmA, tmB, p, s) : launch_conv_e<BN, STAGES, EPI_PLAIN, false, false, SLAB>(tmA, tmB, p, s);
-}
-static int dispatch_conv(int BN, bool slab, const CUtensorMap& tmA, const CUtensorMap& tmB, const TcConvParams& p, cudaStream_t s) {
-  switch (BN * 2 + slab) {
-    case 128: return launch_conv<64, 4, false>(tmA, tmB, p, s, "tc_conv_kernel<64,4>");
-    case 256: return launch_conv<128, 4, false>(tmA, tmB, p, s, "tc_conv_kernel<128,4>");
-    case 129: return launch_conv<64, 4, true>(tmA, tmB, p, s, "tc_conv_kernel<64,4>");
+    case EPI_STATS: return launch_conv_e<BN, STAGES, EPI_STATS, false, false, SLAB, RESB>(tmA, tmB, p, s);
+    case EPI_BNBWD: return launch_conv_e<BN, STAGES, EPI_BNBWD, false, false, SLAB, RESB>(tmA, tmB, p, s);
+    case EPI_ACTBWD: return launch_conv_e<BN, STAGES, EPI_ACTBWD, false, false, SLAB, RESB>(tmA, tmB, p, s);
+  }
+  return (p.scale && p.bias) ? launch_conv_e<BN, STAGES, EPI_PLAIN, true, false, SLAB, RESB>(tmA, tmB, p, s)
+                             : launch_conv_e<BN, STAGES, EPI_PLAIN, false, false, SLAB, RESB>(tmA, tmB, p, s);
+}
+static int dispatch_conv(int BN, bool slab, bool resb, const CUtensorMap& tmA, const CUtensorMap& tmB, const TcConvParams& p, cudaStream_t s) {
+  switch (BN * 4 + slab * 2 + resb) {
+    case 256: return launch_conv<64, 4, false>(tmA, tmB, p, s, "tc_conv_kernel<64,4>");
+    case 512: return launch_conv<128, 4, false>(tmA, tmB, p, s, "tc_conv_kernel<128,4>");
+    case 258: return launch_conv<64, 4, true>(tmA, tmB, p, s, "tc_conv_kernel<64,4>");
+    case 257: return launch_conv<64, 4, false, true>(tmA, tmB, p, s, "tc_conv_kernel<64,4>");
+    case 259: return launch_conv<64, 4, true, true>(tmA, tmB, p, s, "tc_conv_kernel<64,4>");
   }
   return -4;
+}
+static bool resb_tile(const TcConvParams& p, int BN, bool slab) {
+  if (g_tc_test_no_resb || BN != 64 || p.mode != 1) return false;
+  const int units = p.taps_h * p.taps_w * p.chunks;
+  return units <= RESB_UNITS && (long)units * (slab ? 2 : 1) * BN * 128 <= RESB_BYTES;
 }
 static bool slab_tile(const TcConvParams& p, int BN) {
   if (g_tc_test_per_tap || BN != 64 || p.Wt % 8) return false;
@@ -599,7 +654,7 @@
   if (make_map_bf16(&tmA, x, 4, dims, strides, box, es)) return -1;
   p.tiles_m = g.N * g.OH * g.OW / 128; p.tiles_n = g.O / BN; p.phases = 1;
   if (w_mn ? weight_map(&tmB, w, g.C, 1, g.O, 64) : weight_map(&tmB, w, g.O, g.KH * g.KW, g.C, BN)) return -1;
-  return dispatch_conv(BN, slab, tmA, tmB, p, s);
+  return dispatch_conv(BN, slab, false, tmA, tmB, p, s);
 }
 
 int k_tc_dgrad(const ConvGeom& g, const __nv_bfloat16* dy, const __nv_bfloat16* w, const float* bias, __nv_bfloat16* dx, int act, float alpha, cudaStream_t s, const TcEpi* epi) {
@@ -619,7 +674,7 @@
   if (weight_map(&tmB, w, g.O, 16, g.C, 64)) return -1;
   if (make_map_bf16(&tmA, dy, 4, dims, strides, box, es)) return -1;
   p.tiles_m = g.N * g.OH * g.OW / 128; p.tiles_n = g.C / BN; p.phases = 4;
-  return dispatch_conv(BN, slab, tmA, tmB, p, s);
+  return dispatch_conv(BN, slab, resb_tile(p, BN, slab), tmA, tmB, p, s);
 }
 
 bool tc_deconv_ps_shape(const ConvGeom& g) { return is_k4s2p1_geom(g) && g.C >= 1 && g.C <= 4 && g.O % 64 == 0; }
diff --git a/gan_deeplearning4j_b200/engine.py b/gan_deeplearning4j_b200/engine.py
--- a/gan_deeplearning4j_b200/engine.py
+++ b/gan_deeplearning4j_b200/engine.py
@@ -441,7 +441,7 @@
 def test_conv_ex(ctx: Context, kind: int, geom: Dict[str, int], a, b, out_size: int, *, epi: int = 0, act: str = "identity", alpha: float = 0.0,
                  bias=None, scale=None, groups: int = 1, aux=None, aux2=None, iters: int = 1, impl: int = 1, bn: int = 0, max_ctas: int = 0,
                  poison: bool = False, w_mn: bool = False, per_tap: bool = False, info: Optional[dict] = None, defer: bool = False, db=None,
-                 precision: int = BF16, param_offset: int = 0, splits: int = 0):
+                 precision: int = BF16, param_offset: int = 0, splits: int = 0, resb: bool = True):
     g = _lib.ConvGeom(**geom)
     a, b = _f32(a).ravel(), _f32(b).ravel()
     out = np.empty(out_size, np.float32)
@@ -450,6 +450,7 @@
     o.epi, o.act, o.alpha, o.groups = epi, ACTS[act], alpha, groups
     o.bn, o.max_ctas, o.poison, o.w_mn, o.per_tap, o.defer = bn, max_ctas, int(poison), int(w_mn), int(per_tap), int(defer)
     o.param_offset, o.splits = param_offset, splits
+    o.resb = 0 if resb else -1
     if db is not None:
         assert db.dtype == np.float32 and db.flags.c_contiguous
         o.db = _fp(db)
@@ -463,7 +464,7 @@
     ms = C.c_float()
     check(ctx.lib.b2g_test_conv_ex(ctx.h, kind, impl, precision, C.byref(g), _fp(a), _fp(b), _fp(out), iters, C.byref(ms), C.byref(o)))
     if info is not None:
-        info["slab"], info["splits"] = bool(o.slab), o.splits
+        info["slab"], info["resb"], info["splits"] = bool(o.slab), bool(o.resb), o.splits
     return out, stats, o.kernel.decode(), ms.value
 
 
diff --git a/include/b200gan.h b/include/b200gan.h
--- a/include/b200gan.h
+++ b/include/b200gan.h
@@ -193,6 +193,7 @@
   int32_t per_tap;
   int32_t slab;
   int32_t defer;
+  int32_t resb;
   float* db;
   int32_t param_offset;
   int32_t splits;
```
